# anhtu293/nndepth

Hardware: AMD Instinct MI355X
Metric: stereo pairs/sec at 544x960, 32 iters (RAFT-Stereo) (higher is better)
Workload: dtype f32 carried as 2 range-scaled fp16 pieces per operand (3 MFMA products, fp32 accumulate); 1 GPU; RAFT-Stereo base (ctx 64), 544x960, 32 iters, batch 1 per GPU, all 32 up_disp emitted; parallelism=single, launch=direct

## Files before the change

nndepth_amd/csrc/common.h:

```cpp
#pragma once
#include <hip/hip_runtime.h>
#include <atomic>
#include <cstdarg>
#include <cstdio>
#include "../../include/nndepth_amd.h"
#include "split_arith.h"

namespace nnd {

void set_error(const char* fmt, ...);

#define NND_HIP_CHECK(expr)                                                              \
    do {                                                                                 \
        hipError_t _e = (expr);                                                          \
        if (_e != hipSuccess) {                                                          \
            nnd::set_error("%s failed: %s (%s:%d)", #expr, hipGetErrorString(_e), __FILE__, __LINE__); \
            return NND_ERR_HIP;                                                          \
        }                                                                                \
    } while (0)

#define NND_LAUNCH_CHECK()                                                               \
    do {                                                                                 \
        hipError_t _e = hipGetLastError();                                               \
        if (_e != hipSuccess) {                                                          \
            nnd::set_error("kernel launch failed: %s (%s:%d)", hipGetErrorString(_e), __FILE__, __LINE__); \
            return NND_ERR_HIP;                                                          \
        }                                                                                \
    } while (0)

#define NND_REQUIRE(cond, ...)                                                           \
    do {                                                                                 \
        if (!(cond)) {                                                                   \
            nnd::set_error(__VA_ARGS__);                                                 \
            return NND_ERR_INVALID;                                                      \
        }                                                                                \
    } while (0)

#define NND_TRY(x)                           \
    do {                                     \
        if ((rc = (x)) != NND_OK) return rc; \
    } while (0)

template <class Desc>
static inline int check_desc(const Desc* d, unsigned allowed_flags, const char* name) {
    NND_REQUIRE(d, "%s: null descriptor", name);
    NND_REQUIRE(d->struct_size == (int32_t)sizeof(Desc), "%s: descriptor of %d bytes, this library expects %d (struct_size)", name,
                d->struct_size, (int)sizeof(Desc));
    NND_REQUIRE((d->flags & ~allowed_flags) == 0, "%s: unknown flags 0x%x", name, d->flags);
    return NND_OK;
}

struct Switches {
    bool no_fused_upsample, no_fused_lookup, no_fused_flow_branch, no_c4, agcl_v1, no_thin3d, corr_build_v1, corr_build_no_ksplit, igev_squeeze_v1, igev_squeeze_walk, no_folded_flow_head, no_conv1x1_stream,
        conv_verbose, debug_sync;
    int split_ny, split_ks, split_p;
    bool split_no_fast;
    bool no_merged_fb_lookup;
    int conv_p, conv_ks, conv_wco;
    int agcl_pb;
    bool lds_poison_on;
    unsigned lds_poison;
    int lds_slack;
    bool enc_no_c4;
    bool no_slab3d;
    int slab3d_rounds;
};
const Switches& switches();

static inline int raise_lds_limit(const void* kern, std::atomic<unsigned>& done, int bytes = 160 * 1024) {
    int dev = 0;
    NND_HIP_CHECK(hipGetDevice(&dev));
    const unsigned bit = 1u << (dev & 31);
    if (!(done.load(std::memory_order_relaxed) & bit)) {
        NND_HIP_CHECK(hipFuncSetAttribute(kern, hipFuncAttributeMaxDynamicSharedMemorySize, bytes));
        done.fetch_or(bit, std::memory_order_relaxed);
    }
    return NND_OK;
}

bool calibrating();
struct CalibScope {
    explicit CalibScope(bool on);
    ~CalibScope();
    CalibScope(const CalibScope&) = delete;
    CalibScope& operator=(const CalibScope&) = delete;
    bool on;
};
struct Act;
struct Lay;
int calib_amax_act(const Act& a, const Lay& lay, int B, int H, int W, const float* tail, hipStream_t s);
int calib_amax_flat(const float* x, int64_t n, const float* tail, hipStream_t s);
int calib_finish(float* blob, const int64_t* tail_offs, int n, int32_t* status_dev, hipStream_t s);

#ifdef __HIPCC__
__device__ __forceinline__ void fmac_scalar(float& acc, float a, float b) { asm("v_fmac_f32 %0, %1, %2" : "+v"(acc) : "v"(a), "v"(b)); }

__device__ __forceinline__ float relu_nan(float v) { return __builtin_elementwise_maximum(v, 0.f); }
__device__ __forceinline__ float clamp_nan(float v, float lo, float hi) {
    return __builtin_elementwise_minimum(__builtin_elementwise_maximum(v, lo), hi);
}
#endif

int to_tiled(const float* src, float* dst, int64_t dbs, int B, int C, int H, int W, hipStream_t s, int c0 = 0, bool c4 = false);
int from_tiled(const float* src, int64_t sbs, float* dst, int B, int C, int H, int W, hipStream_t s, int c0 = 0, bool c4 = false);

static inline int cdiv(int a, int b) { return (a + b - 1) / b; }
static inline int64_t cdiv64(int64_t a, int64_t b) { return (a + b - 1) / b; }

enum ConvEpilogue {
    EPI_LINEAR = 0,
    EPI_RELU = 1,
    EPI_GRU_ZR = 2,
    EPI_GRU_Q = 3,
    EPI_SCALE = 4,
    EPI_AFFINE = 5,
    EPI_SIGMOID_RANGE = 6,
    EPI_GELU = 7,
    EPI_HSWISH = 8
};

struct ConvLayer {
    int KH, KW, Cin, Cout, CI_T;
    int stride = 1;
    int arith = 0;
    bool range_scaled() const { return split_range_scaled(arith); }
    int64_t s_off = -1;
    int nchunks;
    int ncb;
    int64_t w_off, b_off;
    int64_t w_floats() const {
        return arith ? (int64_t)ncb * nchunks * KH * KW * arith * 256
                     : (int64_t)ncb * nchunks * KH * KW * CI_T * 32;
    }
    int64_t b_floats() const { return (int64_t)ncb * 32 + (range_scaled() ? 4 : 0); }
    double flops(int B, int H, int W) const { return 2.0 * B * H * W * (double)Cout * Cin * KH * KW; }
    int64_t tail_off() const { return b_off + (int64_t)ncb * 32; }
};

struct Act {
    float* ptr;
    int64_t bstride;
    int C;
};

struct ConvIO {
    Act src0, src1;
    Act out0, out1;
    Act aux0, aux1;
    Act bmap;
    int hidden = 0;
    float scale = 1.f;
    int Hin = 0, Win = 0;
    int flags = 0;
    bool src_tiled = false;
    bool dst_tiled = false;
    bool src_c4 = false;
    bool dst_c4 = false;
    int cout_need = 0;
    int force_ks = 0;
};

static inline bool conv_shape_built(int KH, int KW) { return (KH == 1 && (KW == 1 || KW == 5)) || (KW == 1 && KH == 5) || (KH == 3 && KW == 3); }

int conv_ci_t(int KH, int KW, int Cin, int stride = 1, int Cout = 0);

int launch_conv(const ConvLayer& L, const float* blob, const ConvIO& io, int epi,
                int B, int H, int W, hipStream_t stream);

void pack_conv(const ConvLayer& L, int nparts, const float* const* w, const float* const* b,
               const int* cout, float* blob, const int* ci_map = nullptr, int cin_src = 0);

bool conv_split_supported(int KH, int KW, int Cin, int stride, int arith, int Cout = 0);
int launch_conv_split(const ConvLayer& L, const float* blob, const ConvIO& io, int epi, int B, int H, int W, hipStream_t stream);
bool flow_branch_supported(const ConvLayer& f2, int fc);
int launch_flow_branch(const ConvLayer& f2, const float* blob, const float* w7t, const float* b7, const float* flow, int64_t fbs,
                       int fc, const ConvIO& io, int B, int H, int W, hipStream_t stream);
void pack_conv_split(const ConvLayer& L, int nparts, const float* const* w, const float* const* b, const int* cout, float* blob,
                     const int* ci_map, int cin_src);

bool thin3d_supported(int Cout, int stride);
bool slab3d_supported(int Cout, int C0, int C1, int stride, int arith);
int64_t slab3d_packed_floats(int Cout, int Ct, int stride);
void slab3d_pack(int Cout, int Ct, int stride, const float* w, const float* scale, const float* shift, float* out);
int slab3d_forward(int Cout, int C0, int C1, int stride, const float* packed, const float* x0, const float* x1, float* y, int N, int D,
                   int H, int W, float slope, hipStream_t s);
int64_t thin3d_packed_floats(int Cout, int Ct);
void thin3d_pack(int Cout, int Ct, const float* w, const float* scale, const float* shift, float* out);
int thin3d_forward(int Cout, int C0, int C1, int stride, const float* packed, const float* x0, const float* x1, float* y, int N, int D,
                   int H, int W, float slope, hipStream_t s);

int corr1d_lookup_launch(const float* pyr, const float* coords, float* out, int B, int H, int W, int num_levels,
                         int radius, hipStream_t stream, bool tiled);
int group_lookup_flat_launch(const float* pyr, const float* coords, float* out, int B, int G, int H, int W, int num_levels, int radius,
                             hipStream_t stream, bool tiled);
int igev_lookup_launch(const float* feat_pyramid, const float* geo_pyramid, const float* coords, float* out, int B, int G, int H,
                       int W, int num_levels, int radius, hipStream_t stream, bool tiled);
int convex_upsample_launch(const float* flow, const float* mask, float* out, int B, int C, int H, int W, int rate,
                           hipStream_t stream, bool tiled);

int agcl_iter_launch(const float* f1, const float* f2, const float* flow, float* warped, float* out, int N, int C, int H,
                     int W, int small_patch, hipStream_t s, bool tiled);
int agcl_offset_launch(const float* f1, const float* f2, const float* flow, const float* extra, float* out, int N, int C, int H,
                       int W, int small_patch, hipStream_t s, bool tiled);
int agcl_check(const char* what, int N, int C, int H, int W);
bool agcl_offset_cl_supported(int C);
int agcl_offset_cl_launch(const float* f1c, const float* f2c, const float* flow, const float* extra, float* out, int N, int C,
                          int H, int W, int small_patch, hipStream_t s, bool tiled);
int nchw_to_nhwc_launch(const float* in, float* out, int N, int C, int P, hipStream_t s);
int lookup_convc1_launch(const float* pyr, const float* geo, int G, const float* coords, const ConvLayer& L, const float* blob,
                         float* c1, int64_t c1_bs, int B, int H, int W, int num_levels, int radius, hipStream_t stream, bool c1_c4);
bool flow_branch_lookup_supported(int arith);
int flow_branch_lookup_launch(const ConvLayer& f2, const float* blob, const float* w7t, const float* b7, const float* flow, int64_t fbs,
                              int fc, const ConvIO& io, const float* pyr, const float* coords, const ConvLayer& Lc1, float* c1,
                              int64_t c1_bs, int B, int H, int W, int num_levels, int radius, hipStream_t stream, bool c1_c4);
bool igev_lookup_convc1_il_supported(int G, int num_levels, int radius);
int igev_lookup_convc1_il_launch(const float* il, int G, const float* coords, const ConvLayer& L, const float* blob, float* c1,
                                 int64_t c1_bs, int B, int H, int W, int num_levels, int radius, hipStream_t stream, bool c1_c4);
struct MaskUpFlowHead {
    const float* x;
    long xbs;
    int hid;
    const float* w;
    const float* bias;
    const float* coords_in;
    float *coords_out, *flow_out, *delta_out;
    float* hx_flow;
    long hx_bs;
    int hx_pm;
    int absolute;
};

bool mask_upsample_supported(int rate, int cin, int flow_channels);
bool mask_upsample_fold_supported(const ConvLayer& L, int hid);
int mask_upsample_launch(const ConvLayer& L, const float* blob, const float* x, int64_t xbs, const float* flow, float* out,
                         int B, int H, int W, int rate, hipStream_t stream, bool tiled, int flow_channels = 1, bool x_c4 = false,
                         const MaskUpFlowHead* fh = nullptr);

}
```

nndepth_amd/csrc/conv_epilogue.h:

```cpp
#pragma once
#include "common.h"
#include "layout.h"

namespace nnd {

typedef float f32x16 __attribute__((ext_vector_type(16)));

struct ConvArgs {
    const float* src0;
    const float* src1;
    long bs0, bs1;
    int c0, c1;
    const float* wpk;
    const float* bias;
    float* out0;
    float* out1;
    long obs0, obs1;
    const float* aux0;
    const float* aux1;
    long abs0, abs1;
    const float* bmap;
    long bmbs;
    Lay ls, ld;
    int H, W, Cout, nchunks, epi, hidden;
    int Hin, Win;
    int tiles_x, wco, ks, npos, ngroups;
    int flags;
    const float* cscale;
    float scale;
    int dbg_stamp;
};

__device__ __forceinline__ float exp_acc(float x) {
    const float L2E = 1.44269504088896341f;
    x = clamp_nan(x, -87.0f, 88.0f);
    const float t = x * L2E;
    const float r = fmaf(x, 1.92596299e-8f, fmaf(x, L2E, -t));
    const float e = __builtin_amdgcn_exp2f(t);
    return fmaf(e, r * 0.693147180559945f, e);
}
__device__ __forceinline__ float rcp_acc(float d) {
    float y = __builtin_amdgcn_rcpf(d);
    return fmaf(fmaf(-d, y, 1.0f), y, y);
}
__device__ __forceinline__ float sigmoidf_(float v) { return rcp_acc(1.0f + exp_acc(-v)); }
__device__ __forceinline__ float tanhf_(float v) {
    const float ax = fabsf(v);
    const float big = fmaf(-2.0f, rcp_acc(exp_acc(2.0f * ax) + 1.0f), 1.0f);
    const float x2 = ax * ax;
    const float small = ax * fmaf(x2, fmaf(x2, 0.133333333f, -0.333333333f), 1.0f);
    return copysignf(ax < 0.04f ? small : big, v);
}

template <int P>
__device__ __forceinline__ void conv_epilogue_planar(const ConvArgs& a, const f32x16 (&acc)[P], const int cb, const int b, const int h2,
                                                     const int reg0, const int nreg, const int (&ys)[P], const int (&xs)[P]) {
    const int H = a.H, W = a.W;
    const long DP = a.ld.plane;
    const int epi = a.epi;
    float bias_r[16];
#pragma unroll
    for (int reg = 0; reg < 16; ++reg) {
        const int co = cb * 32 + (reg & 3) + 8 * (reg >> 2) + 4 * h2;
        bias_r[reg] = (!a.bmap && reg >= reg0 && reg < reg0 + nreg && co < a.Cout) ? a.bias[co] : 0.f;
    }
#pragma unroll
    for (int pp = 0; pp < P; ++pp) {
        const int y = ys[pp], x = xs[pp];
        const bool pix_ok = (y < H && x < W);
        const long pix = pix_ok ? pix_off(a.ld, y, x) : 0;
        float h_r[16], z_r[16];
        if (a.bmap) {
#pragma unroll
            for (int reg = 0; reg < 16; ++reg) {
                const int co = cb * 32 + (reg & 3) + 8 * (reg >> 2) + 4 * h2;
                const bool ok = pix_ok && reg >= reg0 && reg < reg0 + nreg && co < a.Cout;
                bias_r[reg] = ok ? a.bmap[b * a.bmbs + co * DP + pix] : 0.f;
            }
        }
        if (epi == EPI_AFFINE) {
#pragma unroll
            for (int reg = 0; reg < 16; ++reg) {
                const int co = cb * 32 + (reg & 3) + 8 * (reg >> 2) + 4 * h2;
                const bool ok = pix_ok && reg >= reg0 && reg < reg0 + nreg && co < a.Cout;
                z_r[reg] = ok ? a.cscale[co] : 0.f;
                h_r[reg] = (ok && a.aux0) ? a.aux0[b * a.abs0 + co * DP + pix] : 0.f;
            }
        }
        if (epi == EPI_GRU_ZR || epi == EPI_GRU_Q) {
#pragma unroll
            for (int reg = 0; reg < 16; ++reg) {
                const int co = cb * 32 + (reg & 3) + 8 * (reg >> 2) + 4 * h2;
                const bool ok = pix_ok && reg >= reg0 && reg < reg0 + nreg && co < a.Cout;
                h_r[reg] = 0.f;
                z_r[reg] = 0.f;
                if (epi == EPI_GRU_Q) {
                    if (ok) {
                        h_r[reg] = a.aux0[b * a.abs0 + co * DP + pix];
                        z_r[reg] = a.aux1[b * a.abs1 + co * DP + pix];
                    }
                } else if (ok && co >= a.hidden) {
                    h_r[reg] = a.aux0[b * a.abs0 + (co - a.hidden) * DP + pix];
                }
            }
        }
        if (!pix_ok) continue;
#pragma unroll
        for (int reg = 0; reg < 16; ++reg) {
            if (reg < reg0 || reg >= reg0 + nreg) continue;
            const int co = cb * 32 + (reg & 3) + 8 * (reg >> 2) + 4 * h2;
            if (co >= a.Cout) continue;
            const float v = acc[pp][reg] + bias_r[reg];
            if (epi == EPI_RELU) {
// ... 111 lines not shown
                }
                r0[i] = o0;
                r1[i] = o1;
            }
            const bool to1 = epi == EPI_GRU_ZR && co0 >= a.hidden;
            float* d0 = to1 ? a.out1 + b * a.obs1 + (long)(co0 - a.hidden) * DP + pix : a.out0 + b * a.obs0 + (long)co0 * DP + pix;
            float rr[4];
#pragma unroll
            for (int i = 0; i < 4; ++i) rr[i] = to1 ? r1[i] : r0[i];
            if (full) {
                *reinterpret_cast<float4*>(d0) = make_float4(rr[0], rr[1], rr[2], rr[3]);
                if (epi == EPI_GRU_Q && a.out1) *reinterpret_cast<float4*>(a.out1 + b * a.obs1 + (long)co0 * DP + pix) = make_float4(r1[0], r1[1], r1[2], r1[3]);
            } else {
#pragma unroll
                for (int i = 0; i < 4; ++i)
                    if (co0 + i < a.Cout) {
                        d0[i] = rr[i];
                        if (epi == EPI_GRU_Q && a.out1) a.out1[b * a.obs1 + (long)co0 * DP + pix + i] = r1[i];
                    }
            }
        }
    }
}

template <int P, int NG>
struct EpiOpsC4 {
    float4 bm[P][NG], hv[P][NG], zv[P][NG];
    float4 scale4[NG];
    long pix[P];
    bool pix_ok[P];
};

template <int P, int NG>
__device__ __forceinline__ void epi_c4_load(const ConvArgs& a, const int cb, const int b, const int h2, const int q0,
                                            const int (&ys)[P], const int (&xs)[P], EpiOpsC4<P, NG>& e) {
    const long DP = a.ld.plane;
    const int epi = a.epi;
    auto ld4 = [](const float* p) { return *reinterpret_cast<const float4*>(p); };
    float4 bias4[NG];
#pragma unroll
    for (int j = 0; j < NG; ++j) {
        const int co0 = cb * 32 + 8 * (q0 + j) + 4 * h2;
        float bv[4], sv[4];
#pragma unroll
        for (int i = 0; i < 4; ++i) {
            bv[i] = (!a.bmap && co0 + i < a.Cout) ? a.bias[co0 + i] : 0.f;
            sv[i] = (epi == EPI_AFFINE && co0 + i < a.Cout) ? a.cscale[co0 + i] : 0.f;
        }
        bias4[j] = make_float4(bv[0], bv[1], bv[2], bv[3]);
        e.scale4[j] = make_float4(sv[0], sv[1], sv[2], sv[3]);
    }
#pragma unroll
    for (int pp = 0; pp < P; ++pp) {
        const int y = ys[pp], x = xs[pp];
        const bool pix_ok = (y < a.H && x < a.W);
        const long pix = pix_ok ? pix_off(a.ld, y, x) : 0;
        e.pix_ok[pp] = pix_ok;
        e.pix[pp] = pix;
#pragma unroll
        for (int j = 0; j < NG; ++j) {
            const int co0 = cb * 32 + 8 * (q0 + j) + 4 * h2;
            const bool ok = pix_ok && co0 + 3 < a.Cout;
            const float4 zero = make_float4(0.f, 0.f, 0.f, 0.f);
            e.bm[pp][j] = bias4[j];
            e.hv[pp][j] = zero;
            e.zv[pp][j] = zero;
            if (a.bmap && ok) e.bm[pp][j] = ld4(a.bmap + b * a.bmbs + (long)co0 * DP + pix);
            if (epi == EPI_AFFINE) {
                if (a.aux0 && ok) e.hv[pp][j] = ld4(a.aux0 + b * a.abs0 + (long)co0 * DP + pix);
            } else if (epi == EPI_GRU_Q) {
                if (ok) {
                    e.hv[pp][j] = ld4(a.aux0 + b * a.abs0 + (long)co0 * DP + pix);
                    e.zv[pp][j] = ld4(a.aux1 + b * a.abs1 + (long)co0 * DP + pix);
                }
            } else if (epi == EPI_GRU_ZR) {
                if (ok && co0 >= a.hidden) e.hv[pp][j] = ld4(a.aux0 + b * a.abs0 + (long)(co0 - a.hidden) * DP + pix);
            }
        }
    }
}

template <int P, int NG>
__device__ __forceinline__ void epi_c4_store(const ConvArgs& a, const float4 (&cacc)[P][NG], const int cb, const int b, const int h2,
                                             const int q0, const EpiOpsC4<P, NG>& e) {
    const long DP = a.ld.plane;
    const int epi = a.epi;
    auto get = [](const float4& v, int i) { return i == 0 ? v.x : (i == 1 ? v.y : (i == 2 ? v.z : v.w)); };
#pragma unroll
    for (int pp = 0; pp < P; ++pp) {
        if (!e.pix_ok[pp]) continue;
        const long pix = e.pix[pp];
#pragma unroll
        for (int j = 0; j < NG; ++j) {
            const int co0 = cb * 32 + 8 * (q0 + j) + 4 * h2;
            if (co0 >= a.Cout) continue;
            const bool full = co0 + 3 < a.Cout;
            float r0[4], r1[4];
#pragma unroll
            for (int i = 0; i < 4; ++i) {
                const float ac = get(cacc[pp][j], i);
                const float v = ac + get(e.bm[pp][j], i);
                float o0 = v, o1 = 0.f;
                if (epi == EPI_RELU) o0 = relu_nan(v);
                else if (epi == EPI_SCALE) o0 = a.scale * v;
                else if (epi == EPI_SIGMOID_RANGE) o0 = a.scale * (sigmoidf_(v) - 0.5f) * 2.0f;
                else if (epi == EPI_AFFINE) {
                    float y2 = fmaf(ac, get(e.scale4[j], i), get(e.bm[pp][j], i));
                    if (a.flags & 4) y2 = y2 > 0.f ? y2 : a.scale * y2;
                    if (a.flags & 1) y2 = relu_nan(y2);
                    if (a.aux0) y2 = get(e.hv[pp][j], i) + y2;
                    if (a.flags & 2) y2 = relu_nan(y2);
                    o0 = y2;
                } else if (epi == EPI_GRU_ZR) {
                    const float sg = sigmoidf_(v);
                    o0 = sg;
                    o1 = sg * get(e.hv[pp][j], i);
                } else if (epi == EPI_GRU_Q) {
                    const float qq = tanhf_(v);
                    o0 = fmaf(get(e.zv[pp][j], i), qq, (1.0f - get(e.zv[pp][j], i)) * get(e.hv[pp][j], i));
                    o1 = o0;
                }
                r0[i] = o0;
                r1[i] = o1;
            }
            const bool to1 = epi == EPI_GRU_ZR && co0 >= a.hidden;
            float* d0 = to1 ? a.out1 + b * a.obs1 + (long)(co0 - a.hidden) * DP + pix : a.out0 + b * a.obs0 + (long)co0 * DP + pix;
            float rr[4];
#pragma unroll
            for (int i = 0; i < 4; ++i) rr[i] = to1 ? r1[i] : r0[i];
            if (full) {
                *reinterpret_cast<float4*>(d0) = make_float4(rr[0], rr[1], rr[2], rr[3]);
                if (epi == EPI_GRU_Q && a.out1) *reinterpret_cast<float4*>(a.out1 + b * a.obs1 + (long)co0 * DP + pix) = make_float4(r1[0], r1[1], r1[2], r1[3]);
            } else {
#pragma unroll
                for (int i = 0; i < 4; ++i)
                    if (co0 + i < a.Cout) {
                        d0[i] = rr[i];
                        if (epi == EPI_GRU_Q && a.out1) a.out1[b * a.obs1 + (long)co0 * DP + pix + i] = r1[i];
                    }
            }
        }
    }
}

template <int P>
__device__ __forceinline__ void conv_epilogue(const ConvArgs& a, const f32x16 (&acc)[P], const int cb, const int b, const int h2,
                                              const int reg0, const int nreg, const int (&ys)[P], const int (&xs)[P]) {
    if (a.ld.ci == 4) conv_epilogue_c4<P>(a, acc, cb, b, h2, reg0, nreg, ys, xs);
    else conv_epilogue_planar<P>(a, acc, cb, b, h2, reg0, nreg, ys, xs);
}

}
```

nndepth_amd/csrc/conv_launch.h:

```cpp
#pragma once
#include "common.h"
#include "conv_epilogue.h"
#include "layout.h"

#include <cstring>

namespace nnd {

inline int conv_check_io(const char* who, const ConvLayer& L, const ConvIO& io, int epi, int H, int W, int* Hin, int* Win) {
    NND_REQUIRE(io.src0.C + io.src1.C == L.Cin, "%s: source channels %d+%d != Cin %d", who, io.src0.C, io.src1.C, L.Cin);
    NND_REQUIRE(L.stride == 1 || L.stride == 2, "%s: stride %d not supported", who, L.stride);
    *Hin = io.Hin > 0 ? io.Hin : H, *Win = io.Win > 0 ? io.Win : W;
    NND_REQUIRE(H == (*Hin + L.stride - 1) / L.stride && W == (*Win + L.stride - 1) / L.stride,
                "%s: output %dx%d does not match input %dx%d at stride %d", who, H, W, *Hin, *Win, L.stride);
    NND_REQUIRE(!io.src_c4 || (io.src_tiled && io.src0.C % 4 == 0 && io.src1.C % 4 == 0), "%s: c4 sources need channel counts %% 4 == 0", who);
    NND_REQUIRE(!io.dst_c4 || (io.dst_tiled && (L.Cout % 4 == 0 || (!io.bmap.ptr && !io.aux0.ptr && !io.aux1.ptr && !io.out1.ptr))),
                "%s: c4 destination with per-pixel operands needs Cout %% 4 == 0", who);
    NND_REQUIRE(epi != EPI_AFFINE || L.s_off >= 0, "%s: EPI_AFFINE needs a packed scale vector", who);
    return NND_OK;
}

inline void conv_fill_args(const ConvLayer& L, const float* blob, const ConvIO& io, int epi, int H, int W, int Hin, int Win, ConvArgs* out) {
    ConvArgs& a = *out;
    memset(&a, 0, sizeof(a));
    a.src0 = io.src0.ptr; a.bs0 = io.src0.bstride; a.c0 = io.src0.C;
    a.src1 = io.src1.ptr; a.bs1 = io.src1.bstride; a.c1 = io.src1.C;
    a.wpk = blob + L.w_off; a.bias = blob + L.b_off;
    a.out0 = io.out0.ptr; a.obs0 = io.out0.bstride;
    a.out1 = io.out1.ptr; a.obs1 = io.out1.bstride;
    a.aux0 = io.aux0.ptr; a.abs0 = io.aux0.bstride;
    a.aux1 = io.aux1.ptr; a.abs1 = io.aux1.bstride;
    a.bmap = io.bmap.ptr; a.bmbs = io.bmap.bstride;
    a.ls = make_lay(Hin, Win, io.src_tiled, io.src_c4);
    a.ld = make_lay(H, W, io.dst_tiled, io.dst_c4);
    a.H = H; a.W = W; a.Hin = Hin; a.Win = Win; a.Cout = L.Cout; a.nchunks = L.nchunks; a.epi = epi; a.hidden = io.hidden; a.flags = io.flags;
    a.cscale = L.s_off >= 0 ? blob + L.s_off : nullptr; a.scale = io.scale;
}

template <class CanStage>
inline bool conv_restrict_cout(const ConvLayer& L, int cout_need, int* ny, int* wco, CanStage can_stage) {
    const int nb = cdiv(cout_need, 32);
    if (cout_need <= 0 || nb >= L.ncb) return false;
    const int w = cdiv(nb, *ny), rows = cdiv(nb, *wco);
    if (w < *wco && can_stage(w)) {
        *wco = w;
        *ny = cdiv(nb, w);
        return true;
    }
    if (rows >= *ny) return false;
    *ny = rows;
    return true;
}

}
```

nndepth_amd/csrc/conv_mfma.hip:

```cpp
#include "conv_launch.h"

#include <cmath>
#include <cstdlib>
#include <cstring>
#include <type_traits>

namespace nnd {

#ifndef NND_INTERLEAVE
#define NND_INTERLEAVE 0
#endif

#ifndef NND_SC
#define NND_SC 8
#endif
__host__ __device__ constexpr int patch_stride(int PC, int SC) {
    int s = SC;
    while (s < PC) s += 2 * SC;
    return s;
}

#ifdef NND_DBG_STAMPS
__device__ unsigned long long g_stamps[4096 * 8];
#define NND_STAMP(i)                                                                                   \
// ... 411 lines not shown
                double unit = (double)cdiv(L.nchunks, ks) * P;
                double per_simd = std::ceil(waves / 1024.0);
                double t = (per_simd <= occ) ? per_simd * unit : std::ceil(waves / (1024.0 * occ)) * occ * unit;
                t *= std::ceil(wco * ks / 4.0) * 4.0 / (wco * ks);
                if (waves <= 1024.0) t *= 1.10;
                t *= 1.0 + 0.02 * (4 - wco);
                t *= 1.0 - 0.02 * (P - 1);
                t *= 1.0 + 0.01 * (ks - 1);
                if (t < best) {
                    best = t;
                    *out = {P, wco, ks, tx, ty, npos, ngroups, ne, lds};
                    found = true;
                }
            }
        }
    }
    return found;
}

template <int KH, int KW, int CI_T, int P, int NE, int STR = 1>
static int launch_one(const ConvArgs& a, const TileCfg& cfg, hipStream_t stream) {
    auto kern = conv_mfma_kernel<KH, KW, CI_T, P, NE, STR>;
    if (cfg.lds > 64 * 1024) {
        static std::atomic<unsigned> raised{0};
        if (int rc = raise_lds_limit(reinterpret_cast<const void*>(kern), raised)) return rc;
    }
    hipLaunchKernelGGL(kern, cfg.grid, cfg.block, cfg.lds, stream, a);
    return NND_OK;
}

template <int KH, int KW, int CI_T>
static int launch_shape(const ConvArgs& a, const TileCfg& cfg, hipStream_t stream) {
    return cfg.ne <= 8 ? launch_one<KH, KW, CI_T, 1, 8>(a, cfg, stream) : launch_one<KH, KW, CI_T, 1, 16>(a, cfg, stream);
}

static bool plan_tile(const ConvLayer& L, const ConvIO& io, int epi, int B, int H, int W, TileCfg* cfg) {
    if (!pick_tile(L, io.src0.C, io.src1.C, B, H, W, cfg, io.force_ks)) return false;
    cfg->stream1x1 = !switches().no_conv1x1_stream && L.KH == 1 && L.KW == 1 && L.stride == 1 && io.src1.C == 0 && io.src_tiled &&
                     (!io.dst_c4 || L.Cout % 4 == 0) && !io.bmap.ptr && (L.Cin == 64 || L.Cin == 96 || L.Cin == 128) &&
                     (epi == EPI_LINEAR || epi == EPI_RELU || epi == EPI_SCALE || epi == EPI_AFFINE);
    if (cfg->stream1x1) {
        cfg->grid = dim3((unsigned)cdiv64((long)L.ncb * cfg->tiles_x * cfg->tiles_y, 4), 1, B), cfg->block = dim3(256);
        return true;
    }
    auto groups = [&](int wco) { return 64 * wco * cfg->ks / cfg->npos; };
    int ny = cdiv(L.ncb, cfg->wco);
    cfg->restricted = conv_restrict_cout(L, io.cout_need, &ny, &cfg->wco,
                                         [&](int wco) { return groups(wco) > 0 && cdiv(cfg->ks * L.CI_T, groups(wco)) <= 16; });
    cfg->ngroups = groups(cfg->wco), cfg->ne = cdiv(cfg->ks * L.CI_T, cfg->ngroups);
    cfg->grid = dim3(cfg->tiles_x * cfg->tiles_y, ny, B), cfg->block = dim3(64 * cfg->wco * cfg->ks);
    return true;
}

static int check_tile_plan(const ConvLayer& L, const TileCfg& cfg) {
    const int SR_ = 32 / NND_SC, st = L.stride;
    const int PR_ = (SR_ - 1) * st + L.KH, PC_ = (cfg.P * NND_SC - 1) * st + L.KW;
    const size_t patch = (size_t)st * st * ((PR_ + st - 1) / st) * patch_stride((PC_ + st - 1) / st, NND_SC);
    NND_REQUIRE(cfg.lds >= ((size_t)2 * cfg.ks * L.CI_T * patch + 1) * sizeof(float) &&
                    (cfg.ks == 1 || cfg.lds >= (size_t)cfg.wco * cfg.ks * cfg.P * 1024 * sizeof(float)) && cfg.lds <= 160 * 1024,
                "conv: LDS plan %zu B does not cover the patch buffers / split-K tiles", cfg.lds);
    NND_REQUIRE(cfg.npos == PR_ * PC_ && cfg.npos * cfg.ngroups <= 64 * cfg.wco * cfg.ks && cfg.ngroups * cfg.ne >= cfg.ks * L.CI_T && cfg.ne <= 16,
                "conv: staging plan (%d positions x %d groups x %d) does not cover %d channels", cfg.npos, cfg.ngroups, cfg.ne, cfg.ks * L.CI_T);
    return NND_OK;
}

static void print_tile_plan(const ConvLayer& L, const ConvIO& io, const TileCfg& cfg) {
    if (cfg.stream1x1)
        fprintf(stderr, "[nnd] conv1x1_stream Cin=%d Cout=%d CI_T=%d: grid %ux1x%d%s\n", L.Cin, L.Cout, L.CI_T, cfg.grid.x, (int)cfg.grid.z,
                io.dst_c4 ? ", c4 destination" : "");
    else
        fprintf(stderr, "[nnd] conv %dx%d Cin=%d Cout=%d CI_T=%d: P=%d, wco=%d, ks=%d, ne=%d, grid %ux%ux%u, lds %zu B%s%s\n",
                L.KH, L.KW, L.Cin, L.Cout, L.CI_T, cfg.P, cfg.wco, cfg.ks, cfg.ne, cfg.grid.x, cfg.grid.y, cfg.grid.z, cfg.lds,
                io.cout_need > 0 ? (cfg.restricted ? ", restricted to the wanted output channels" : ", whole layer (not restrictable)") : "",
                L.stride == 2 ? ", stride 2" : "");
}

int launch_conv(const ConvLayer& L, const float* blob, const ConvIO& io, int epi, int B, int H, int W, hipStream_t stream) {
    if (L.arith != 0) {
        NND_REQUIRE(epi != EPI_GELU && epi != EPI_HSWISH, "conv: EPI_GELU / EPI_HSWISH are built on the exact fp32 kernel only");
        return launch_conv_split(L, blob, io, epi, B, H, W, stream);
    }
    int rc, Hin, Win;
    NND_TRY(conv_check_io("conv", L, io, epi, H, W, &Hin, &Win));
    NND_REQUIRE(io.src1.C == 0 || io.src0.C % L.CI_T == 0, "conv: first source (%d ch) must be a multiple of %d", io.src0.C, L.CI_T);
    NND_REQUIRE(!io.src_c4 || L.stride == 1, "conv: c4 sources need stride 1");
    NND_REQUIRE((long)(L.Cin + 2 * L.CI_T) * tiled_plane(Hin, Win) < (1L << 31), "conv: plane offsets exceed 32 bits");
    NND_REQUIRE((epi != EPI_GELU && epi != EPI_HSWISH) || (!io.dst_c4 && !io.out1.ptr && !io.bmap.ptr),
                "conv: EPI_GELU / EPI_HSWISH are built for a planar out0 only");
    TileCfg cfg;
    NND_REQUIRE(plan_tile(L, io, epi, B, H, W, &cfg),
                "conv: no tile configuration for %dx%d Cin=%d Cout=%d stride %d (NND_CONV_CFG p=%d ks=%d wco=%d, layer ks=%d)", L.KH, L.KW,
                L.Cin, L.Cout, L.stride, switches().conv_p, switches().conv_ks, switches().conv_wco, io.force_ks);
    NND_TRY(check_tile_plan(L, cfg));
    ConvArgs a;
    conv_fill_args(L, blob, io, epi, H, W, Hin, Win, &a);
    a.tiles_x = cfg.tiles_x; a.wco = cfg.wco; a.ks = cfg.ks; a.npos = cfg.npos; a.ngroups = cfg.ngroups;
    if (switches().conv_verbose) print_tile_plan(L, io, cfg);
    const int ntiles = cfg.tiles_x * cfg.tiles_y, KQ = L.nchunks * L.CI_T / 8, KH = L.KH, KW = L.KW, CI_T = L.CI_T;
    rc = NND_ERR_UNSUPPORTED;
    if (cfg.stream1x1) {
        rc = NND_OK;
        if (L.Cin == 64) launch_conv1x1_stream<8>(a, cfg.grid, ntiles, L.ncb, KQ, stream);
        else if (L.Cin == 96) launch_conv1x1_stream<12>(a, cfg.grid, ntiles, L.ncb, KQ, stream);
        else launch_conv1x1_stream<16>(a, cfg.grid, ntiles, L.ncb, KQ, stream);
    } else if (L.stride == 2) {
        if (KH == 3 && KW == 3 && CI_T == 16) rc = launch_one<3, 3, 16, 1, 16, 2>(a, cfg, stream);
        else if (KH == 1 && KW == 1 && CI_T == 16) rc = launch_one<1, 1, 16, 1, 16, 2>(a, cfg, stream);
        else set_error("conv %dx%d stride 2 CI_T=%d not instantiated", KH, KW, CI_T);
    } else if (KH == 1 && KW == 1 && CI_T == 128) rc = launch_shape<1, 1, 128>(a, cfg, stream);
    else if (KH == 1 && KW == 1 && CI_T == 32) rc = launch_shape<1, 1, 32>(a, cfg, stream);
    else if (KH == 3 && KW == 3 && CI_T == 32) rc = launch_shape<3, 3, 32>(a, cfg, stream);
    else if (KH == 3 && KW == 3 && CI_T == 16) rc = launch_shape<3, 3, 16>(a, cfg, stream);
    else if (KH == 1 && KW == 5 && CI_T == 32) rc = launch_shape<1, 5, 32>(a, cfg, stream);
    else if (KH == 5 && KW == 1 && CI_T == 32) rc = launch_shape<5, 1, 32>(a, cfg, stream);
    else if (KH == 1 && KW == 5 && CI_T == 64) rc = launch_shape<1, 5, 64>(a, cfg, stream);
    else if (KH == 5 && KW == 1 && CI_T == 64) rc = launch_shape<5, 1, 64>(a, cfg, stream);
    else set_error("conv %dx%d CI_T=%d not instantiated", KH, KW, CI_T);
    if (rc != NND_OK) return rc;
    NND_LAUNCH_CHECK();
    return NND_OK;
}

int conv_ci_t(int KH, int KW, int Cin, int stride, int Cout) {
    if (stride == 2) return 16;
    if (KH == 3 && KW == 3 && Cin <= 64) return 16;
    if (KH * KW == 5 && Cin >= 256 && Cout >= 256) return 64;
    return (KH == 1 && KW == 1 && Cin >= 128) ? 128 : 32;
}

void pack_conv(const ConvLayer& L, int nparts, const float* const* w, const float* const* bvec,
               const int* cout, float* blob, const int* ci_map, int cin_src) {
    if (L.arith != 0) return pack_conv_split(L, nparts, w, bvec, cout, blob, ci_map, cin_src);
    if (!ci_map) cin_src = L.Cin;
    const int NT = L.KH * L.KW, NQ = L.CI_T / 8;
    float* wp = blob + L.w_off;
    float* bp = blob + L.b_off;
    memset(wp, 0, sizeof(float) * L.w_floats());
    memset(bp, 0, sizeof(float) * L.b_floats());
    int co0 = 0;
    for (int part = 0; part < nparts; ++part) {
        for (int col = 0; col < cout[part]; ++col) {
            int co = co0 + col;
            int cb = co / 32, i = co % 32;
            bp[co] = bvec[part] ? bvec[part][col] : 0.f;
            for (int ci = 0; ci < L.Cin; ++ci) {
                int chunk = ci / L.CI_T, cl = ci % L.CI_T;
                int pair = cl / 2, h2 = cl % 2;
                int q = pair / 4, j = pair % 4;
                int lane = h2 * 32 + i;
                for (int t = 0; t < NT; ++t) {
                    size_t idx = (((((size_t)cb * L.nchunks + chunk) * NT + t) * NQ + q) * 64 + lane) * 4 + j;
                    wp[idx] = w[part][((size_t)col * cin_src + (ci_map ? ci_map[ci] : ci)) * NT + t];
                }
            }
        }
        co0 += cout[part];
    }
}

#ifdef NND_DBG_STAMPS
extern "C" int nnd_debug_read_stamps(unsigned long long* host, int n) {
    return hipMemcpyFromSymbol(host, HIP_SYMBOL(g_stamps), sizeof(unsigned long long) * n) == hipSuccess ? 0 : -1;
}
#endif
}
```

nndepth_amd/csrc/conv_split.hip:

```cpp
#include "conv_launch.h"
#include "conv_split_kernel.h"
#include "flow_branch.h"

#include <atomic>
#include <cmath>
#include <cstdlib>
#include <cstring>

namespace nnd {

namespace {
uint16_t f16_rn(float x) {
    const _Float16 h = (_Float16)x;
    uint16_t u;
    memcpy(&u, &h, 2);
    return u;
}
float f16_to_f(uint16_t u) {
    _Float16 h;
    memcpy(&h, &u, 2);
    return (float)h;
}
uint16_t bf16_rn(float x) {
    uint32_t u;
    memcpy(&u, &x, 4);
    if ((u & 0x7fffffffu) > 0x7f800000u) return (uint16_t)((u >> 16) | 0x40);
    u += 0x7fffu + ((u >> 16) & 1u);
    return (uint16_t)(u >> 16);
}
float bf16_to_f(uint16_t h) {
    const uint32_t u = (uint32_t)h << 16;
    float f;
    memcpy(&f, &u, 4);
    return f;
}

bool pick_split(const ConvLayer& L, int c0, int c1, int B, int H, int W, bool fast_ok, SplitCfg* out) {
    const int NS = L.arith, STR = L.stride;
    const int npos = split_patch(L.KH, L.KW, NS, STR).NPOS;
    const size_t subb = split_patch(L.KH, L.KW, NS, STR).SUBB;
    int tiles_x, ntiles = split_tiles(H, W, &tiles_x);
    int force_ny = switches().split_ny, force_ks = switches().split_ks, force_p = switches().split_p;
    const bool forced = force_ny > 0 || force_ks > 0 || force_p > 0;
    const long px_wgs2 = (long)cdiv(ntiles, 2) * B;
    bool rule = false;
    if (L.nchunks <= 4 && !forced && L.ncb <= SPLIT_MAX_WAVES) {
        force_ny = 1;
        while (force_ny < L.ncb && (L.ncb % force_ny != 0 || L.ncb / force_ny > 4)) ++force_ny;
        force_ks = 1;
        force_p = 2;
        rule = true;
    }
    bool try_ks2 = false;
    if (!rule && px_wgs2 >= 448 && !forced) {
        rule = true;
        force_ks = 1;
        force_ny = 1;
        force_p = 2;
        const int max_wco = L.nchunks >= 16 ? 4 : SPLIT_MAX_WAVES;
        while (force_ny < L.ncb && (L.ncb % force_ny != 0 || L.ncb / force_ny > max_wco)) ++force_ny;
        try_ks2 = px_wgs2 * force_ny * (L.ncb / force_ny) < 256 * SPLIT_MAX_WAVES / 2;
    }
    auto search = [&](int f_ny, int f_ks, int f_p) {
        double best = 1e30;
        bool found = false;
        for (int P : {2, 3, 4}) {
            if ((f_p > 0 && P != f_p) || (f_p <= 0 && P != 2)) continue;
            const long px_wgs = (long)cdiv(ntiles, P) * B;
            for (int ny = 1; ny <= L.ncb; ++ny) {
                if (L.ncb % ny != 0 || (f_ny > 0 && ny != f_ny)) continue;
                const int wco = L.ncb / ny;
                for (int ks : {1, 2, 4}) {
                    if (f_ks > 0 && ks != f_ks) continue;
                    const int waves = wco * ks;
                    if (waves > SPLIT_MAX_WAVES || ks > L.nchunks) continue;
                    if (c1 > 0 && c0 % (ks * 16) != 0) continue;
                    const bool fast = fast_ok && L.nchunks % ks == 0;
                    if (P > 2) continue;
                    if (STR == 2 && !fast) continue;
                    const int nu = split_staging_units(P, npos, ks, waves);
                    if (nu > 4 || (P == 3 && nu > 3)) continue;
                    size_t lds = (size_t)2 * ks * P * subb;
                    const size_t red = ks > 1 ? (size_t)waves * P * 4096 : 0;
                    if (red > lds) lds = red;
                    if (lds > 160 * 1024) continue;
                    const int max_waves = P > 2 ? 8 : SPLIT_MAX_WAVES;
                    int wg_per_cu = (int)((160 * 1024) / lds);
                    if (wg_per_cu > max_waves / waves) wg_per_cu = max_waves / waves;
                    if (wg_per_cu < 1) wg_per_cu = 1;
                    const double rounds = std::ceil((double)px_wgs * ny / (256.0 * wg_per_cu));
                    const double simd_waves = std::ceil(waves * wg_per_cu / 4.0);
                    double t = rounds * simd_waves * cdiv(L.nchunks, ks) * P / 2.0;
                    t *= 1.0 + 0.03 * (ks - 1);
                    t *= 1.0 + 0.02 * (4 - (wco < 4 ? wco : 4));
                    if (nu > 2 && P == 2) t *= 1.2;
                    if (t < best) {
                        best = t;
                        *out = {ny, wco, ks, P, ntiles, tiles_x, split_nu_variant(nu), fast, lds, STR};
                        found = true;
                    }
                }
            }
        }
        return found;
    };
    if (try_ks2 && search(force_ny, 2, force_p)) return true;
    if (search(force_ny, force_ks, force_p)) return true;
    return rule && search(-1, -1, -1);
}

bool restrict_split(const ConvLayer& L, int cout_need, SplitCfg* cfg) {
    const int npos = split_patch(L.KH, L.KW, L.arith, L.stride).NPOS;
    auto units = [&](int wco) { return split_staging_units(cfg->P, npos, cfg->ks, wco * cfg->ks); };
    if (!conv_restrict_cout(L, cout_need, &cfg->ny, &cfg->wco, [&](int wco) { return cfg->P == 2 && units(wco) <= 4; })) return false;
    cfg->nu = split_nu_variant(units(cfg->wco));
    return true;
}

bool split_fast_ok(const ConvLayer& L) { return !switches().split_no_fast || L.stride == 2; }
bool plan_split(const ConvLayer& L, const ConvIO& io, int B, int H, int W, SplitCfg* cfg) {
    if (!pick_split(L, io.src0.C, io.src1.C, B, H, W, split_fast_ok(L), cfg)) return false;
    cfg->restricted = restrict_split(L, io.cout_need, cfg);
    cfg->grid = dim3(cdiv(cfg->ntiles, cfg->P), cfg->ny, B), cfg->block = dim3(64 * cfg->wco * cfg->ks);
    return true;
}

void print_split_plan(const ConvLayer& L, const ConvIO& io, const SplitCfg& cfg) {
    fprintf(stderr, "[nnd] conv_split %dx%d Cin=%d Cout=%d pieces=%d: ny=%d, wco=%d, ks=%d, P=%d, nu=%d%s, grid %ux%ux%u, lds %zu B%s%s\n", L.KH,
            L.KW, L.Cin, L.Cout, L.arith, cfg.ny, cfg.wco, cfg.ks, cfg.P, cfg.nu, cfg.fast ? ", fast" : "", cfg.grid.x, cfg.grid.y, cfg.grid.z, cfg.lds,
            io.cout_need > 0 ? (cfg.restricted ? ", restricted to the wanted output channels" : ", whole layer (not restrictable)") : "",
            L.stride == 2 ? ", stride 2" : "");
}
}

extern template int launch_split_ns<1>(const ConvArgs&, const SplitCfg&, int, int, hipStream_t);
extern template int launch_split_ns<2>(const ConvArgs&, const SplitCfg&, int, int, hipStream_t);
extern template int launch_split_ns<3>(const ConvArgs&, const SplitCfg&, int, int, hipStream_t);

bool conv_split_supported(int KH, int KW, int Cin, int stride, int arith, int Cout) {
    if ((arith != 3 && arith != 2 && arith != 1) || (stride != 1 && stride != 2) || Cin % 16 != 0) return false;
    if (stride == 2) return ((KH == 3 && KW == 3) || (KH == 1 && KW == 1)) && Cout >= 96;
    return conv_shape_built(KH, KW);
}

int launch_conv_split(const ConvLayer& L, const float* blob, const ConvIO& io, int epi, int B, int H, int W, hipStream_t stream) {
    int rc, Hin, Win;
    NND_REQUIRE(conv_split_supported(L.KH, L.KW, L.Cin, L.stride, L.arith, L.Cout), "conv_split: %dx%d Cin=%d Cout=%d stride %d arith %d not built",
                L.KH, L.KW, L.Cin, L.Cout, L.stride, L.arith);
    NND_TRY(conv_check_io("conv_split", L, io, epi, H, W, &Hin, &Win));
    NND_REQUIRE(L.CI_T == 16 && L.nchunks * 16 == L.Cin, "conv_split: layer was not planned for 16-channel chunks");
    NND_REQUIRE(L.stride == 1 || io.src1.C == 0, "conv_split: stride 2 is built for one source");
    NND_REQUIRE((long)(L.Cin + 64) * tiled_plane(Hin, Win) < (1L << 31), "conv_split: plane offsets exceed 32 bits");
    SplitCfg cfg;
    NND_REQUIRE(plan_split(L, io, B, H, W, &cfg),
                "conv_split: no configuration for %dx%d Cin=%d (%d+%d) Cout=%d stride %d (NND_SPLIT_CFG ny=%d ks=%d P=%d%s)", L.KH, L.KW,
                L.Cin, io.src0.C, io.src1.C, L.Cout, L.stride, switches().split_ny, switches().split_ks, switches().split_p,
                split_fast_ok(L) ? "" : ", NND_SPLIT_NO_FAST");
    ConvArgs a;
    conv_fill_args(L, blob, io, epi, H, W, Hin, Win, &a);
    a.tiles_x = cfg.tiles_x; a.wco = cfg.wco; a.ks = cfg.ks; a.npos = cfg.ntiles;
#ifdef NND_DBG_STAMPS
    {
        static std::atomic<int> launches{0};
        static const int only = getenv("NND_DBG_STAMP_LAUNCH") ? atoi(getenv("NND_DBG_STAMP_LAUNCH")) : -1;
        const int idx = launches.fetch_add(1);
        a.dbg_stamp = only < 0 || idx == only;
    }
#endif
    if (calibrating() && split_range_scaled(L.arith))
        for (const Act* src : {&io.src0, &io.src1}) NND_TRY(calib_amax_act(*src, a.ls, B, Hin, Win, blob + L.tail_off(), stream));
    if (switches().conv_verbose) print_split_plan(L, io, cfg);
    rc = L.arith == 3   ? launch_split_ns<3>(a, cfg, L.KH, L.KW, stream)
         : L.arith == 2 ? launch_split_ns<2>(a, cfg, L.KH, L.KW, stream)
                        : launch_split_ns<1>(a, cfg, L.KH, L.KW, stream);
    NND_REQUIRE(rc != NND_ERR_UNSUPPORTED, "conv_split: shape %dx%d P=%d nu=%d %s is not instantiated", L.KH, L.KW, cfg.P, cfg.nu, cfg.fast ? "fast" : "generic");
    if (rc != NND_OK) return rc;
    NND_LAUNCH_CHECK();
    return NND_OK;
}

void pack_conv_split(const ConvLayer& L, int nparts, const float* const* w, const float* const* bvec, const int* cout, float* blob,
                     const int* ci_map, int cin_src) {
    if (!ci_map) cin_src = L.Cin;
    const int NT = L.KH * L.KW, NS = L.arith;
    uint16_t* wp = reinterpret_cast<uint16_t*>(blob + L.w_off);
    float* bp = blob + L.b_off;
    memset(wp, 0, sizeof(float) * L.w_floats());
    memset(bp, 0, sizeof(float) * L.b_floats());
    const bool f16 = split_range_scaled(NS);
    float wscale = 1.f;
    if (f16) {
        float wmax = 0.f;
        for (int part = 0; part < nparts; ++part)
            for (int col = 0; col < cout[part]; ++col)
                for (int ci = 0; ci < L.Cin; ++ci)
                    for (int t = 0; t < NT; ++t) {
                        const float v = std::fabs(w[part][((size_t)col * cin_src + (ci_map ? ci_map[ci] : ci)) * NT + t]);
                        if (std::isfinite(v) && v > wmax) wmax = v;
                    }
        int e = 0;
        if (wmax > 0.f) std::frexp(wmax, &e);
        const int s = wmax > 0.f ? 14 - e : 0;
        wscale = std::ldexp(1.f, s);
        float* tail = bp + L.ncb * 32;
        tail[SPLIT_TAIL_OSCALE] = std::ldexp(1.f, -(s + SPLIT_F16_XSHIFT));
        tail[SPLIT_TAIL_XSCALE] = std::ldexp(1.f, SPLIT_F16_XSHIFT);
        tail[SPLIT_TAIL_AMAX] = 0.f;
        tail[SPLIT_TAIL_WSINV] = std::ldexp(1.f, -s);
    }
    int co0 = 0;
    for (int part = 0; part < nparts; ++part) {
        for (int col = 0; col < cout[part]; ++col) {
            const int co = co0 + col, cb = co / 32, i = co % 32;
            bp[co] = bvec[part] ? bvec[part][col] : 0.f;
            for (int ci = 0; ci < L.Cin; ++ci) {
                const int chunk = ci / 16, cl = ci % 16, h = cl / 8, j = cl % 8, lane = h * 32 + i;
                for (int t = 0; t < NT; ++t) {
                    float res = w[part][((size_t)col * cin_src + (ci_map ? ci_map[ci] : ci)) * NT + t] * wscale;
                    for (int s = 0; s < NS; ++s) {
                        const uint16_t piece = f16 ? f16_rn(res) : bf16_rn(res);
                        res -= f16 ? f16_to_f(piece) : bf16_to_f(piece);
                        wp[((((((size_t)cb * L.nchunks + chunk) * NT + t) * NS + s) * 64 + lane) * 8) + j] = piece;
                    }
                }
            }
        }
        co0 += cout[part];
    }
}

template <int FC, int NS>
static int launch_fb(const FlowBranchArgs& a, dim3 grid, dim3 block, hipStream_t stream) {
    auto kern = flow_branch_kernel<FC, NS>;
    static std::atomic<unsigned> raised{0};
    if (int rc = raise_lds_limit(reinterpret_cast<const void*>(kern), raised)) return rc;
    const size_t lds = (size_t)(fb_lds_bytes<FC, NS>()) + switches().lds_slack;
    hipLaunchKernelGGL(kern, grid, block, lds, stream, a);
    return NND_OK;
}

bool flow_branch_supported(const ConvLayer& f2, int fc) {
    return (f2.arith == 3 || f2.arith == 2 || f2.arith == 1) && f2.KH == 3 && f2.KW == 3 && f2.Cin == FB_C1 && f2.Cout == 64 && f2.stride == 1 && (fc == 1 || fc == 2);
}
// ... 41 lines not shown
```

nndepth_amd/csrc/conv_split_kernel.h:

```cpp
#pragma once
#include "common.h"
#include "conv_epilogue.h"
#include "layout.h"
#include "split_arith.h"

#include <type_traits>
#include <utility>

namespace nnd {

#ifndef NND_SPLIT_BSLOTS
#define NND_SPLIT_BSLOTS 2
#endif

#ifdef NND_DBG_STAMPS
static __device__ unsigned long long g_split_stamps[4096 * 8];
#define NND_SSTAMP(i)                                                                                  \
    do {                                                                                               \
        if (threadIdx.x == 0 && a.dbg_stamp) {                                                         \
            const unsigned lin_ = blockIdx.x + gridDim.x * (blockIdx.y + gridDim.y * blockIdx.z);      \
            if (lin_ < 4096) g_split_stamps[lin_ * 8 + (i)] = __builtin_amdgcn_s_memrealtime();        \
        }                                                                                              \
    } while (0)
#define NND_SCLOCK(i)                                                                                  \
    do {                                                                                               \
        if (threadIdx.x == 0 && a.dbg_stamp) {                                                         \
            const unsigned lin_ = blockIdx.x + gridDim.x * (blockIdx.y + gridDim.y * blockIdx.z);      \
            if (lin_ < 4096) g_split_stamps[lin_ * 8 + (i)] = __builtin_amdgcn_s_memtime();            \
        }                                                                                              \
    } while (0)
#else
#define NND_SSTAMP(i)
#define NND_SCLOCK(i)
#endif
#if defined(NND_DBG_STAMPS) && defined(NND_DBG_PROLOGUE)
#undef NND_SCLOCK
#define NND_SCLOCK(i)
#define NND_PSTAMP(i) NND_SSTAMP(i)
#else
#define NND_PSTAMP(i)
#endif

__host__ __device__ constexpr int split_pos_bytes(int NS) { return NS * 32 + 16; }
__host__ __device__ constexpr int split_row_bytes(int PC, int NS) {
    int rb = (PC * split_pos_bytes(NS) + 15) / 16;
    while (rb % 16 != 8) ++rb;
    return rb * 16;
}

__device__ __forceinline__ int lane_pixel(int l31) {
    const bool g0 = (l31 < 4) || (l31 >= 12 && l31 < 16) || (l31 >= 20 && l31 < 28);
    const int idx = g0 ? (l31 < 4 ? l31 : (l31 < 16 ? l31 - 8 : l31 - 12)) : (l31 < 12 ? l31 - 4 : (l31 < 20 ? l31 - 8 : l31 - 16));
    return (g0 ? 0 : 16) + idx;
}

__host__ __device__ constexpr int split_gcd(int a, int b) { return b == 0 ? a : split_gcd(b, a % b); }

template <int N, typename F, int... I>
__device__ __forceinline__ void split_static_for_impl(F&& f, std::integer_sequence<int, I...>) {
    (f(std::integral_constant<int, I>{}), ...);
}
template <int N, typename F>
__device__ __forceinline__ void split_static_for(F&& f) {
    split_static_for_impl<N>(static_cast<F&&>(f), std::make_integer_sequence<int, N>{});
}

struct SplitPatch {
    int PRI, PCI, NPH, PRP, PCP, NPOS, PS, ROWB, PHB, SUBB;
};
__host__ __device__ constexpr SplitPatch split_patch(int KH, int KW, int NS, int STR) {
    const int PRI = 3 * STR + KH, PCI = 7 * STR + KW;
    const int NPH = STR == 1 ? 1 : (KH * KW == 1 ? 1 : 4);
    const int PRP = STR == 1 ? PRI : (KH == 1 ? 4 : (PRI + 1) / 2);
    const int PCP = STR == 1 ? PCI : (KW == 1 ? 8 : (PCI + 1) / 2);
    const int NPOS = STR == 1 ? PRI * PCI : (KH * KW == 1 ? 32 : PRI * PCI);
    const int ROWB = split_row_bytes(PCP, NS);
    return {PRI, PCI, NPH, PRP, PCP, NPOS, split_pos_bytes(NS), ROWB, PRP * ROWB, NPH * PRP * ROWB};
}
template <int KH, int KW, int NS, int STR>
struct SplitGeom {
    static constexpr SplitPatch G = split_patch(KH, KW, NS, STR);
    static constexpr int PRI = G.PRI, PCI = G.PCI, NPH = G.NPH, PRP = G.PRP, PCP = G.PCP, NPOS = G.NPOS;
    static constexpr int PS = G.PS, ROWB = G.ROWB, PHB = G.PHB, SUBB = G.SUBB;
};
__host__ __device__ constexpr int split_staging_units(int P, int npos, int ks, int waves) { return (P * npos * 2 * ks + 64 * waves - 1) / (64 * waves); }
__host__ __device__ constexpr int split_nu_variant(int nu) { return nu <= 2 ? 2 : 4; }

__host__ __device__ constexpr int split_pipe_spu(int nunit, int nsteps, int ul) {
    int v = 1;
    while (v < nsteps && nunit - 1 - (nsteps + v - 1) / v < ul + 3) ++v;
    return v;
}
template <int NT, int P, int NU>
struct SplitPipe {
    static constexpr int NUNIT = NT * P, NSTEPS = NU * 4 + 3, UL = 1;
    static constexpr int SPU = split_pipe_spu(NUNIT, NSTEPS, UL), U0 = NUNIT - 1 - (NSTEPS + SPU - 1) / SPU;
    static constexpr bool ON = NT >= 5 && P == 2;
};

template <int KH, int KW, int NS, int P, int NU, bool FAST, bool SRC4, int AD_, int MAXT, int STR = 1>
__global__ void __launch_bounds__(MAXT) conv_split_kernel(ConvArgs a) {
    static_assert(STR == 1 || (FAST && (KH * KW == 9 || KH * KW == 1)), "stride 2: 3x3 / 1x1, FAST regime");
    using Geo = SplitGeom<KH, KW, NS, STR>;
    constexpr int NT = KH * KW, PH = KH / 2, PW = KW / 2;
    constexpr int PC = Geo::PCI, NPOS = Geo::NPOS;
#ifndef NND_SPLIT_NO_PIPE
    constexpr bool PIPE = FAST && SRC4 && SplitPipe<NT, P, NU>::ON && NS != 1;
#else
    constexpr bool PIPE = false;
#endif
    constexpr int PS = Geo::PS, ROWB = Geo::ROWB, SUBB = Geo::SUBB, PHB = Geo::PHB;
    extern __shared__ __attribute__((aligned(16))) unsigned char lds_raw[];
    NND_SSTAMP(0);

    const int tid = threadIdx.x, lane = tid & 63, nthreads = blockDim.x;
    const int wave = __builtin_amdgcn_readfirstlane(tid >> 6);
    const int wco = a.wco, ks = a.ks;
    const int cbi = wave % wco, kj = wave / wco;
    const int h2 = lane >> 5, l31 = lane & 31;
    const int pxl = lane_pixel(l31), r = pxl >> 3, c = pxl & 7;
    const int cb = blockIdx.y * wco + cbi;
    const bool active = cb * 32 < a.Cout;
    const int b = blockIdx.z;
    const int Hin = a.Hin, Win = a.Win;
    const long SP = a.ls.plane;
    const int SCH = ks * 16;
    float oscale = 1.f, xscale = 1.f;
    if constexpr (split_range_scaled(NS)) {
        const float* tail = a.bias + (((a.Cout + 31) >> 5) << 5);
        oscale = tail[SPLIT_TAIL_OSCALE];
        xscale = tail[SPLIT_TAIL_XSCALE];
    }

    int ty0[P], tx0[P];
#pragma unroll
    for (int pp = 0; pp < P; ++pp) {
        const int t = blockIdx.x * P + pp;
        const bool valid = t < a.npos;
        ty0[pp] = valid ? (t / a.tiles_x) * 4 : (1 << 20);
        tx0[pp] = valid ? (t % a.tiles_x) * 8 : 0;
    }

    const int nunits = P * NPOS * 2 * ks;
    int goff[NU], loff[NU], cho[NU];
    bool inimg[NU], own[NU];
#pragma unroll
    for (int i = 0; i < NU; ++i) {
        const int u = PIPE ? min(tid + i * nthreads, nunits - 1) : tid + i * nthreads;
        own[i] = u < nunits;
        const int pos = u % NPOS, rest = u / NPOS;
        const int pp = rest % P, oct = rest / P;
        int pr, pc, lpos;
        if constexpr (STR == 1) {
            pr = pos / PC;
            pc = pos - pr * PC;
            lpos = pr * ROWB + pc * PS;
        } else if constexpr (KH * KW == 1) {
            pr = (pos >> 3) * 2;
            pc = (pos & 7) * 2;
            lpos = (pos >> 3) * ROWB + (pos & 7) * PS;
        } else {
            pr = pos / PC;
            pc = pos - pr * PC;
            lpos = ((pr & 1) * 2 + (pc & 1)) * PHB + (pr >> 1) * ROWB + (pc >> 1) * PS;
        }
        int gy = 0, gx = 0;
#pragma unroll
        for (int q = 0; q < P; ++q)
            if (q == pp) {
                gy = ty0[q] * STR + pr - PH;
                gx = tx0[q] * STR + pc - PW;
            }
        inimg[i] = own[i] && gy >= 0 && gy < Hin && gx >= 0 && gx < Win;
        goff[i] = inimg[i] ? (int)pix_off(a.ls, gy, gx) : 0;
        loff[i] = (oct >> 1) * (P * SUBB) + pp * SUBB + lpos + (oct & 1) * 16;
        cho[i] = oct * 8;
        if constexpr (FAST) goff[i] = inimg[i] ? cho[i] * (int)SP + goff[i] : 0;
        if constexpr (PIPE) goff[i] = cho[i] * (int)SP + (int)pix_off(a.ls, min(max(gy, 0), Hin - 1), min(max(gx, 0), Win - 1));
    }

    NND_PSTAMP(5);
    f32x16 acc[P];
#pragma unroll
    for (int pp = 0; pp < P; ++pp)
#pragma unroll
        for (int i = 0; i < 16; ++i) acc[pp][i] = 0.f;

    const int nchunks = a.nchunks;
    const int nsuper = (nchunks + ks - 1) / ks;
    const uint4* wbase = reinterpret_cast<const uint4*>(a.wpk) + (size_t)(active ? cb : 0) * nchunks * (NT * NS * 64) + lane;
    float stage[NU][8];

    auto chunk_src = [&](int K, const float*& src, int& climit) {
        const int cbase = K * SCH;
        if constexpr (FAST) {
            const bool first = cbase < a.c0;
            const float* s0 = a.src0 + b * a.bs0 + (long)cbase * SP;
            const float* s1 = a.src1 + b * a.bs1 + (long)(cbase - a.c0) * SP;
            src = first ? s0 : s1;
            climit = SCH;
        } else if (cbase < a.c0) {
            src = a.src0 + b * a.bs0 + (long)cbase * SP;
            climit = a.c0 - cbase;
        } else {
            const int cc = cbase - a.c0;
            src = a.src1 + b * a.bs1 + (long)cc * SP;
            climit = a.c1 - cc;
        }
    };
    const bool c4s = FAST ? SRC4 : a.ls.ci == 4;
    auto load_unit = [&](int K, int i) {
        const float* src;
        int climit;
        chunk_src(K, src, climit);
        if constexpr (FAST && SRC4) {
#pragma unroll
            for (int g = 0; g < 2; ++g) {
                const float4 t = *reinterpret_cast<const float4*>(src + (unsigned)(goff[i] + ((PIPE || inimg[i]) ? 4 * g * (int)SP : 0)));
                stage[i][4 * g] = t.x; stage[i][4 * g + 1] = t.y; stage[i][4 * g + 2] = t.z; stage[i][4 * g + 3] = t.w;
            }
        } else if constexpr (FAST) {
            const int step = inimg[i] ? (int)SP : 0;
#pragma unroll
            for (int j = 0; j < 8; ++j) stage[i][j] = src[(unsigned)(goff[i] + j * step)];
        } else if (c4s) {
#pragma unroll
            for (int g = 0; g < 2; ++g) {
                const int ci = cho[i] + 4 * g;
                const float4 t = *reinterpret_cast<const float4*>(src + ((inimg[i] && ci < climit) ? (unsigned)(ci * (int)SP + goff[i]) : 0u));
                stage[i][4 * g] = t.x; stage[i][4 * g + 1] = t.y; stage[i][4 * g + 2] = t.z; stage[i][4 * g + 3] = t.w;
            }
        } else {
#pragma unroll
            for (int j = 0; j < 8; ++j) {
                const int ci = cho[i] + j;
                stage[i][j] = src[(inimg[i] && ci < climit) ? (unsigned)(ci * (int)SP + goff[i]) : 0u];
            }
        }
    };
    auto store_unit = [&](int K, int i) {
        const float* src;
        int climit;
        chunk_src(K, src, climit);
        unsigned char* buf = lds_raw + (K & 1) * (ks * P * SUBB);
        float v[8];
#pragma unroll
        for (int j = 0; j < 8; ++j) v[j] = (inimg[i] && (FAST || cho[i] + j < climit)) ? stage[i][j] : 0.f;
        uint4 pieces[NS];
        split_pieces<NS>(v, pieces, xscale);
        if (own[i]) {
#pragma unroll
            for (int s = 0; s < NS; ++s) *reinterpret_cast<uint4*>(buf + loff[i] + s * 32) = pieces[s];
        }
    };
    auto load_x = [&](int K) {
#pragma unroll
        for (int i = 0; i < NU; ++i) load_unit(K, i);
    };
    auto store_x = [&](int K) {
#pragma unroll
        for (int i = 0; i < NU; ++i) store_unit(K, i);
    };
    auto a_ptr = [&](int K) {
        int ch = K * ks + kj;
        ch = ch < nchunks ? ch : 0;
        return wbase + (size_t)ch * (NT * NS * 64);
    };
    auto load_a = [&](uint4 (&dst)[NS], const uint4* wc, int t) {
#pragma unroll
        for (int s = 0; s < NS; ++s) dst[s] = wc[(t * NS + s) * 64];
    };

    const int lane_base = kj * (P * SUBB) + r * ROWB + c * PS + h2 * 16;

    constexpr int AD = (AD_ < NT ? AD_ : NT), NA = AD + 1;
    uint4 abuf[NA][NS];
#pragma unroll
    for (int g = 0; g < AD; ++g) load_a(abuf[g], a_ptr(0), g);
    load_x(0);
    NND_PSTAMP(6);
    store_x(0);
    NND_PSTAMP(7);
    __syncthreads();
    NND_SSTAMP(1);
    NND_SCLOCK(5);

    uint4 bq2[2][NS];
    uint32_t pw[NU][NS][4];
    auto read_b2 = [&](const unsigned char* xb, int u, uint4 (&dst)[NS]) {
        const int t = u / P, pp = u % P;
        const int dy = t / KW, dx = t % KW;
        const int toff = STR == 1 ? dy * ROWB + dx * PS : ((dy & 1) * 2 + (dx & 1)) * PHB + (dy >> 1) * ROWB + (dx >> 1) * PS;
#pragma unroll
        for (int s = 0; s < NS; ++s) dst[s] = *reinterpret_cast<const uint4*>(xb + pp * SUBB + toff + s * 32);
    };
    auto micro = [&](int q, unsigned char* wbuf) {
        using PP = SplitPipe<NT, P, NU>;
        if (q >= PP::NSTEPS) return;
        if (q < NU * 4) {
            const int i = q / 4, pr = q % 4;
            if constexpr (NS == 2) {
                const float sc = inimg[i] ? xscale : 0.f;
                uint32_t hi, lo;
                asm("v_fma_mixlo_f16 %0, %2, %3, 0\n\t"
                    "v_fma_mixhi_f16 %0, %2, %4, 0\n\t"
                    "v_fma_mixlo_f16 %1, %2, %3, -%0 op_sel_hi:[0,0,1]\n\t"
                    "v_fma_mixhi_f16 %1, %2, %4, -%0 op_sel:[0,0,1] op_sel_hi:[0,0,1]"
                    : "=&v"(hi), "=&v"(lo)
                    : "v"(sc), "v"(stage[i][2 * pr]), "v"(stage[i][2 * pr + 1]));
                pw[i][0][pr] = hi;
                pw[i][1][pr] = lo;
            } else {
                float r0 = inimg[i] ? stage[i][2 * pr] : 0.f, r1 = inimg[i] ? stage[i][2 * pr + 1] : 0.f;
#pragma unroll
                for (int sp = 0; sp < NS; ++sp) {
                    typedef __bf16 v2 __attribute__((ext_vector_type(2)));
                    v2 v;
                    v[0] = (__bf16)r0; v[1] = (__bf16)r1;
                    r0 -= (float)v[0]; r1 -= (float)v[1];
                    pw[i][sp][pr] = __builtin_bit_cast(uint32_t, v);
                }
            }
        }
        const int w = q - 4;
        if (w >= 0 && w / 4 < NU && w % 4 < NS) {
#ifdef NND_SPLIT_NO_LDSW
            if (pw[w / 4][0][0] == 0x12345678u)
#endif
            *reinterpret_cast<uint4*>(wbuf + loff[w / 4] + (w % 4) * 32) =
                make_uint4(pw[w / 4][w % 4][0], pw[w / 4][w % 4][1], pw[w / 4][w % 4][2], pw[w / 4][w % 4][3]);
        }
    };
    auto chunk_pipe = [&](int K, auto par_c, auto more_c) {
        using PP = SplitPipe<NT, P, NU>;
        constexpr int par = decltype(par_c)::value;
        constexpr bool more = decltype(more_c)::value;
        constexpr int NUNIT = PP::NUNIT;
        const int BUFB = ks * P * SUBB;
        const uint4* wc = a_ptr(K);
        const uint4* wn = a_ptr(more ? K + 1 : K);
        const unsigned char* xb = lds_raw + (K & 1) * BUFB + lane_base;
        const unsigned char* xbn = lds_raw + ((K + 1) & 1) * BUFB + lane_base;
        unsigned char* wbuf = lds_raw + ((K + 1) & 1) * BUFB;
#pragma unroll
        for (int t = 0; t < NT; ++t) {
            uint4(&ac)[NS] = abuf[(par + t) % NA];
            uint4(&an)[NS] = abuf[(par + t + AD) % NA];
#ifndef NND_SPLIT_NO_ALOAD
            if (t + AD < NT) load_a(an, wc, t + AD);
            else load_a(an, wn, t + AD - NT);
#else
            for (int s = 0; s < NS; ++s) an[s] = ac[s];
#endif
#pragma unroll
            for (int pp = 0; pp < P; ++pp) {
                const int u = t * P + pp;
#ifndef NND_SPLIT_NO_BREAD
                if (u + 1 < NUNIT) read_b2(xb, u + 1, bq2[(u + 1) & 1]);
                else if (more) read_b2(xbn, 0, bq2[0]);
#endif
                __builtin_amdgcn_sched_barrier(0);
#ifndef NND_SPLIT_NO_MFMA
                split_mfma_step<NS>(ac, bq2[u & 1], acc[pp]);
#else
// ... 38 lines not shown
            for (int s = 0; s < NS; ++s)
                dst[s] = *reinterpret_cast<const uint4*>(xb + pp * SUBB + toff + s * 32);
        };
#pragma unroll
        for (int u = 0; u < NSLOT - 1 && u < NUNIT; ++u) read_b(u, bq[u]);
#pragma unroll
        for (int t = 0; t < NT; ++t) {
            uint4(&ac)[NS] = abuf[(par + t) % NA];
            uint4(&an)[NS] = abuf[(par + t + AD) % NA];
#ifndef NND_SPLIT_NO_ALOAD
            if (t + AD < NT) load_a(an, wc, t + AD);
            else load_a(an, wn, t + AD - NT);
#else
            for (int s = 0; s < NS; ++s) an[s] = ac[s];
#endif
#pragma unroll
            for (int pp = 0; pp < P; ++pp) {
                const int u = t * P + pp;
                if (u + NSLOT - 1 < NUNIT) read_b(u + NSLOT - 1, bq[(u + NSLOT - 1) % NSLOT]);
#ifndef NND_SPLIT_NO_PIN
                if constexpr (FAST) __builtin_amdgcn_sched_barrier(0);
#endif
#ifndef NND_SPLIT_NO_MFMA
                if constexpr (mine)
#else
                if (mine && acc[0][0] == 123.f)
#endif
                    split_mfma_step<NS>(ac, bq[u % NSLOT], acc[pp]);
#ifndef NND_SPLIT_NO_PIN
                if constexpr (FAST) __builtin_amdgcn_sched_barrier(0);
#endif
            }
        }
#ifndef NND_SPLIT_NO_STAGE
        if (more) store_x(K + 1);
#endif
        __syncthreads();
    };
    auto chunk = [&](int K, auto par_c) {
        if constexpr (FAST) {
            chunk_body(K, par_c, std::true_type{});
        } else {
            if (K * ks + kj < nchunks) chunk_body(K, par_c, std::true_type{});
            else chunk_body(K, par_c, std::false_type{});
        }
    };
    constexpr int STEP = NT % NA, PERIOD = NA / split_gcd(STEP, NA);
    if constexpr (PIPE) read_b2(lds_raw + lane_base, 0, bq2[0]);
    if constexpr (PIPE) {
        const int last = nsuper - 1;
        for (int K0 = 0; K0 < last; K0 += PERIOD)
            split_static_for<PERIOD>([&](auto j) {
                constexpr int jj = decltype(j)::value;
                if (jj == 0 || K0 + jj < last) chunk_pipe(K0 + jj, std::integral_constant<int, (jj * STEP) % NA>{}, std::true_type{});
            });
        split_static_for<PERIOD>([&](auto j) {
            constexpr int jj = decltype(j)::value;
            if (PERIOD == 1 || last % PERIOD == jj) chunk_pipe(last, std::integral_constant<int, (jj * STEP) % NA>{}, std::false_type{});
        });
    } else {
        for (int K0 = 0; K0 < nsuper; K0 += PERIOD)
            split_static_for<PERIOD>([&](auto j) {
                constexpr int jj = decltype(j)::value;
                if (jj == 0 || K0 + jj < nsuper) chunk(K0 + jj, std::integral_constant<int, (jj * STEP) % NA>{});
            });
    }

    NND_SSTAMP(2);
    NND_SCLOCK(6);
    if constexpr (split_range_scaled(NS)) {
#pragma unroll
        for (int pp = 0; pp < P; ++pp)
#pragma unroll
            for (int i = 0; i < 16; ++i) acc[pp][i] *= oscale;
    }
    int ys[P], xs[P];
#pragma unroll
    for (int pp = 0; pp < P; ++pp) {
        ys[pp] = ty0[pp] + r;
        xs[pp] = tx0[pp] + c;
    }
    float* red_all = reinterpret_cast<float*>(lds_raw);
    constexpr int TS = P * 1024;
    auto exchange = [&]() {
        if (active) {
            float* red = red_all + (size_t)(cbi * ks + kj) * TS + lane;
#pragma unroll
            for (int pp = 0; pp < P; ++pp)
#pragma unroll
                for (int reg = 0; reg < 16; ++reg) red[pp * 1024 + reg * 64] = acc[pp][reg];
        }
        __syncthreads();
    };
    auto finish_c4 = [&](auto ng_c) {
        constexpr int NG = decltype(ng_c)::value;
        const int q0 = kj * NG;
        EpiOpsC4<P, NG> eo;
#ifndef NND_SPLIT_NO_EPI
        if (active) epi_c4_load<P, NG>(a, cb, b, h2, q0, ys, xs, eo);
#endif
        exchange();
        if (!active) return;
        float4 cacc[P][NG];
#pragma unroll
        for (int pp = 0; pp < P; ++pp)
#pragma unroll
            for (int j = 0; j < NG; ++j) {
                float v[4];
#pragma unroll
                for (int i = 0; i < 4; ++i) {
                    const float* red = red_all + (size_t)(cbi * ks) * TS + pp * 1024 + (4 * (q0 + j) + i) * 64 + lane;
                    float sum = red[0];
#pragma unroll
                    for (int sl = 1; sl < 4 / NG; ++sl) sum += red[(size_t)sl * TS];
                    v[i] = sum;
                }
                cacc[pp][j] = make_float4(v[0], v[1], v[2], v[3]);
            }
        NND_SSTAMP(3);
#ifdef NND_SPLIT_NO_EPI
        if (cacc[0][0].x != 123.456f) return;
#endif
        epi_c4_store<P, NG>(a, cacc, cb, b, h2, q0, eo);
    };
    if (a.ld.ci == 4) {
        if (ks == 4) finish_c4(std::integral_constant<int, 1>{});
        else if (ks == 2) finish_c4(std::integral_constant<int, 2>{});
        else {
            if (!active) return;
            NND_SSTAMP(3);
#ifdef NND_SPLIT_NO_EPI
            if (acc[0][0] != 123.456f) return;
#endif
            conv_epilogue_c4<P>(a, acc, cb, b, h2, 0, 16, ys, xs);
        }
    } else {
        if (ks > 1) exchange();
        if (!active) return;
        const int nreg = 16 / ks, reg0 = kj * nreg;
        if (ks > 1) {
            const float* red = red_all + (size_t)(cbi * ks) * TS + lane;
#pragma unroll
            for (int pp = 0; pp < P; ++pp)
#pragma unroll
                for (int reg = 0; reg < 16; ++reg) {
                    if (reg < reg0 || reg >= reg0 + nreg) continue;
                    float sum = red[pp * 1024 + reg * 64];
                    for (int j = 1; j < ks; ++j) sum += red[(size_t)j * TS + pp * 1024 + reg * 64];
                    acc[pp][reg] = sum;
                }
        }
        NND_SSTAMP(3);
#ifdef NND_SPLIT_NO_EPI
        if (acc[0][0] != 123.456f) return;
#endif
        conv_epilogue_planar<P>(a, acc, cb, b, h2, reg0, nreg, ys, xs);
    }
#ifdef NND_DBG_STAMPS
    __builtin_amdgcn_s_waitcnt(0);
#endif
    NND_SSTAMP(4);
}

struct SplitCfg {
    int ny, wco, ks, P, ntiles, tiles_x, nu;
    bool fast;
    size_t lds;
    int stride;
    bool restricted;
    dim3 grid, block;
};

constexpr int SPLIT_MAX_WAVES = 12;

inline int split_tiles(int H, int W, int* tiles_x) { return (*tiles_x = cdiv(W, 8)) * cdiv(H, 4); }

template <int KH, int KW, int NS, int P, int NU, bool FAST, bool SRC4, int AD, int MAXT, int STR = 1>
int launch_split_kernel(const ConvArgs& a, dim3 grid, dim3 block, size_t lds, hipStream_t stream) {
    auto kern = conv_split_kernel<KH, KW, NS, P, NU, FAST, SRC4, AD, MAXT, STR>;
    if ((int)block.x > MAXT) {
        set_error("conv_split: %u threads exceed the %d-thread bound of this instantiation", block.x, MAXT);
        return NND_ERR_INVALID;
    }
    lds += switches().lds_slack;
    if (lds > 64 * 1024) {
        static std::atomic<unsigned> raised{0};
        if (int rc = raise_lds_limit(reinterpret_cast<const void*>(kern), raised)) return rc;
    }
    hipLaunchKernelGGL(kern, grid, block, lds, stream, a);
    return NND_OK;
}

template <int KH, int KW, int NS>
constexpr int split_fast_ad() {
#ifdef NND_SPLIT_FAST_AD
    return NND_SPLIT_FAST_AD;
#else
    return KH * KW == 9 ? 2 : (KH * KW == 5 ? (NS <= 2 ? 4 : 2) : 1);
#endif
}

template <int KH, int KW, int NS, bool FAST, bool SRC4, int STR>
int launch_split_nu(const ConvArgs& a, const SplitCfg& cfg, hipStream_t stream) {
    constexpr int AD = FAST ? split_fast_ad<KH, KW, NS>() : 1;
    if (split_nu_variant(cfg.nu) == 2) return launch_split_kernel<KH, KW, NS, 2, 2, FAST, SRC4, AD, 768, STR>(a, cfg.grid, cfg.block, cfg.lds, stream);
    return launch_split_kernel<KH, KW, NS, 2, 4, FAST, SRC4, AD, 768, STR>(a, cfg.grid, cfg.block, cfg.lds, stream);
}
template <int KH, int KW, int NS>
int launch_split_shape(const ConvArgs& a, const SplitCfg& cfg, hipStream_t stream) {
    if (cfg.P != 2) return NND_ERR_UNSUPPORTED;
    const bool src4 = a.ls.ci == 4;
    if (cfg.stride == 2) {
        if constexpr (KH * KW == 9 || KH * KW == 1) {
            if (!cfg.fast) return NND_ERR_UNSUPPORTED;
            return src4 ? launch_split_nu<KH, KW, NS, true, true, 2>(a, cfg, stream) : launch_split_nu<KH, KW, NS, true, false, 2>(a, cfg, stream);
        } else {
            return NND_ERR_UNSUPPORTED;
        }
    }
    if (!cfg.fast) return launch_split_nu<KH, KW, NS, false, false, 1>(a, cfg, stream);
    return src4 ? launch_split_nu<KH, KW, NS, true, true, 1>(a, cfg, stream) : launch_split_nu<KH, KW, NS, true, false, 1>(a, cfg, stream);
}

template <int NS>
int launch_split_ns(const ConvArgs& a, const SplitCfg& cfg, int KH, int KW, hipStream_t stream) {
    if (KH == 3 && KW == 3) return launch_split_shape<3, 3, NS>(a, cfg, stream);
    if (KH == 1 && KW == 5) return launch_split_shape<1, 5, NS>(a, cfg, stream);
    if (KH == 5 && KW == 1) return launch_split_shape<5, 1, NS>(a, cfg, stream);
    if (KH == 1 && KW == 1) return launch_split_shape<1, 1, NS>(a, cfg, stream);
    return NND_ERR_UNSUPPORTED;
}

}
```

nndepth_amd/csrc/error.cpp:

```cpp
#include "common.h"

#include <cstdlib>

namespace nnd {
static thread_local char g_err[512] = "";
void set_error(const char* fmt, ...) {
    va_list ap;
    va_start(ap, fmt);
    vsnprintf(g_err, sizeof(g_err), fmt, ap);
    va_end(ap);
}

static Switches g_sw;
static void load_switches() {
    Switches s{};
    auto on = [](const char* n) { return getenv(n) != nullptr; };
    s.no_fused_upsample = on("NND_NO_FUSED_UPSAMPLE");
    s.no_fused_lookup = on("NND_NO_FUSED_LOOKUP");
    s.no_fused_flow_branch = on("NND_NO_FUSED_FLOW_BRANCH");
    s.no_c4 = on("NND_NO_C4");
    s.agcl_v1 = on("NND_AGCL_V1");
    s.no_thin3d = on("NND_NO_THIN3D");
    s.corr_build_v1 = on("NND_CORR_BUILD_V1");
    s.corr_build_no_ksplit = on("NND_CORR_BUILD_NO_KSPLIT");
    s.igev_squeeze_v1 = on("NND_IGEV_SQUEEZE_V1");
    s.igev_squeeze_walk = on("NND_IGEV_SQUEEZE_WALK");
    s.no_folded_flow_head = on("NND_NO_FOLDED_FLOW_HEAD");
    s.no_conv1x1_stream = on("NND_NO_CONV1X1_STREAM");
    s.conv_verbose = on("NND_CONV_VERBOSE");
    s.debug_sync = on("NND_DEBUG_SYNC");
    s.split_ny = s.split_ks = s.split_p = -1;
    if (const char* e = getenv("NND_SPLIT_CFG")) sscanf(e, "%d,%d,%d", &s.split_ny, &s.split_ks, &s.split_p);
    s.split_no_fast = on("NND_SPLIT_NO_FAST");
    s.no_merged_fb_lookup = on("NND_NO_MERGED_FB_LOOKUP");
    s.conv_p = s.conv_ks = s.conv_wco = -1;
    if (const char* e = getenv("NND_CONV_CFG")) sscanf(e, "%d,%d,%d", &s.conv_p, &s.conv_ks, &s.conv_wco);
    if (const char* e = getenv("NND_CONV_P")) s.conv_p = atoi(e);
    s.agcl_pb = getenv("NND_AGCL_PB") ? atoi(getenv("NND_AGCL_PB")) : 0;
    s.lds_poison_on = on("NND_DEBUG_LDS_POISON");
    s.lds_poison = s.lds_poison_on ? (unsigned)strtoul(getenv("NND_DEBUG_LDS_POISON"), nullptr, 0) : 0u;
    s.lds_slack = getenv("NND_DEBUG_LDS_SLACK") ? atoi(getenv("NND_DEBUG_LDS_SLACK")) : 0;
    s.enc_no_c4 = on("NND_ENC_NO_C4");
    s.no_slab3d = on("NND_NO_SLAB3D");
    s.slab3d_rounds = getenv("NND_SLAB3D_ROUNDS") ? atoi(getenv("NND_SLAB3D_ROUNDS")) : 0;
    g_sw = s;
}
namespace {
struct SwitchInit {
    SwitchInit() { load_switches(); }
} g_switch_init;
}
const Switches& switches() { return g_sw; }
}

extern "C" {
int nnd_reload_switches(void) {
    nnd::load_switches();
    return NND_OK;
}
int nnd_version(void) { return NND_VERSION; }
const char* nnd_last_error(void) { return nnd::g_err; }
int nnd_device_count(void) {
    int n = 0;
    if (hipGetDeviceCount(&n) != hipSuccess) {
        (void)hipGetLastError();
        return 0;
    }
    return n;
}
}
```

nndepth_amd/csrc/mask_upsample.hip:

```cpp
#include "common.h"

#include <type_traits>
#include "layout.h"
#include "split_arith.h"

namespace nnd {

typedef float f32x16 __attribute__((ext_vector_type(16)));

#ifdef NND_DBG_STAMPS
__device__ unsigned long long g_mu_stamps[4096 * 8];
#define NND_MSTAMP(i)                                                                             \
    do {                                                                                          \
        if (threadIdx.x == 0 && blockIdx.x < 4096) g_mu_stamps[blockIdx.x * 8 + (i)] = __builtin_amdgcn_s_memrealtime(); \
    } while (0)
#else
#define NND_MSTAMP(i)
#endif

struct MaskUpArgs {
    const float* x;
    long xbs;
    const float* wpk;
    const float* bias;
    const float* flow;
    float* out;
    int H, W, tiles_x, fc;
    Lay lay;
    int x_c4;
    int lds_floats;
    MaskUpFlowHead fh;
};

template <int RATE, int CIN>
struct MaskUpCfg {
    static constexpr int COUT = 9 * RATE * RATE;
    static constexpr int NCB = (COUT + 31) / 32;
    static constexpr int CBW = NCB >= 12 ? 3 : 1;
    static constexpr int G = (NCB + CBW - 1) / CBW;
    static constexpr int NWAVES = 2 * G;
    static constexpr int NT = 64 * NWAVES;
    static constexpr int NST = CIN / 32;
    static constexpr int MT_STRIDE = 33;
    static constexpr int XS_FLOATS = CIN * 32 * 3 / 2;
    static constexpr int LDS_FLOATS = (XS_FLOATS > COUT * MT_STRIDE ? XS_FLOATS : COUT * MT_STRIDE) + 128;
};

template <int RATE, int CIN, int NS = 0, int FHW = 0>
__global__ void __launch_bounds__((MaskUpCfg<RATE, CIN>::NT + 64 * FHW)) mask_upsample_kernel(MaskUpArgs a) {
    constexpr bool SPLIT = NS != 0;
    using Cfg = MaskUpCfg<RATE, CIN>;
    constexpr int COUT = Cfg::COUT, NCB = Cfg::NCB, CBW = Cfg::CBW, G = Cfg::G, NT = Cfg::NT, NST = Cfg::NST;
    constexpr int CI_T = 128;
    constexpr int NCHUNK = CIN / CI_T;
    constexpr int MTS = Cfg::MT_STRIDE;
    static_assert(CIN % 128 == 0 && NST % 2 == 0, "CIN must be a multiple of 128");
    extern __shared__ float lds[];
    NND_MSTAMP(0);
    float* xs = lds;
    float* mt = lds;
    float* fp = lds + a.lds_floats - 128;

    const int tid = threadIdx.x, lane = tid & 63;
    const int wave = __builtin_amdgcn_readfirstlane(tid >> 6);
    const int g = wave % G, kj = wave / G;
    const int h2 = lane >> 5, l31 = lane & 31;
    const int tx0 = (blockIdx.x % a.tiles_x) * 8, ty0 = (blockIdx.x / a.tiles_x) * 4;
    const int b = blockIdx.z;
    const int H = a.H, W = a.W;
    const long HW = (long)H * W;
    const long XP = a.lay.plane;
    float oscale = 1.f, xscale = 1.f;
    if constexpr (split_range_scaled(NS)) {
        oscale = a.bias[Cfg::NCB * 32 + SPLIT_TAIL_OSCALE];
        xscale = a.bias[Cfg::NCB * 32 + SPLIT_TAIL_XSCALE];
    }

    float fh_state = 0.f, fh_bias = 0.f;
    auto fh_finish = [&](float* fbase, int t0) {
        if (t0 >= 60) return;
        const float* part = fbase + a.fh.hid * 105;
        const int pr = t0 / 10, pc = t0 % 10;
        const int y = ty0 + pr - 1, x = tx0 + pc - 1;
        float sum = 0.f;
#pragma unroll
        for (int sl = 0; sl < 16; ++sl) sum += part[sl * 64 + t0];
        sum += fh_bias;
        const bool in = y >= 0 && y < H && x >= 0 && x < W;
        const float cnew = fh_state + sum;
        const float fl = a.fh.absolute ? cnew : cnew - (float)x;
        fp[t0] = in ? fl : 0.f;
        if (in && pr >= 1 && pr <= 4 && pc >= 1 && pc <= 8) {
            const long pix = pix_off(a.lay, y, x);
            a.fh.delta_out[b * XP + pix] = sum;
            a.fh.coords_out[b * XP + pix] = cnew;
            a.fh.flow_out[b * XP + pix] = fl;
            a.fh.hx_flow[b * a.fh.hx_bs + pix * a.fh.hx_pm] = fl;
        }
    };
    constexpr int NQ4 = (CIN / 4 * 32 + NT - 1) / NT;
    float4 v4[SPLIT ? NQ4 : 1];
    if constexpr (SPLIT) {
        const float* src = a.x + b * a.xbs;
#pragma unroll
        for (int i = 0; i < NQ4; ++i) {
            const int e = min(tid, NT - 1) + i * NT;
            const int qd = e >> 5, px = e & 31;
            const int y = ty0 + (px >> 3), x = tx0 + (px & 7);
            const bool ok = e < CIN / 4 * 32 && y < H && x < W;
            if (a.x_c4) {
                v4[i] = *reinterpret_cast<const float4*>(src + (ok ? (unsigned)(qd * 4 * (int)XP + 4 * (int)pix_off(a.lay, y, x)) : 0u));
            } else {
                const unsigned o = ok ? (unsigned)(qd * 4 * (int)XP + (int)pix_off(a.lay, y, x)) : 0u;
                v4[i] = make_float4(src[o], src[ok ? o + (unsigned)XP : 0u], src[ok ? o + 2u * (unsigned)XP : 0u], src[ok ? o + 3u * (unsigned)XP : 0u]);
            }
        }
    }
    if constexpr (FHW > 0) {
        if (tid >= NT) {
            float* fbase = lds + Cfg::LDS_FLOATS;
            const int hid = a.fh.hid, fw_ = __builtin_amdgcn_readfirstlane((tid - NT) >> 6), cn = hid / FHW, c0 = fw_ * cn;
            float* patch = fbase;
            float* fw = fbase + hid * 96;
            const float* src = a.fh.x + b * a.fh.xbs;
            constexpr int NPL = 12, NWL = 5;
            const int total = 96 * (cn / 4), nwt = cn * 9;
            float4 pv[NPL];
            bool pok[NPL];
            float wreg[NWL];
#pragma unroll
            for (int k = 0; k < NWL; ++k) wreg[k] = a.fh.w[c0 * 9 + min(lane + 64 * k, nwt - 1)];
            if (tid - NT < 60) {
                fh_bias = a.fh.bias[0];
                const int y = ty0 + (tid - NT) / 10 - 1, x = tx0 + (tid - NT) % 10 - 1;
                if (y >= 0 && y < H && x >= 0 && x < W) fh_state = a.fh.coords_in[b * XP + pix_off(a.lay, y, x)];
            }
#pragma unroll
            for (int j = 0; j < NPL; ++j) {
                const int e = min(lane + 64 * j, total - 1);
                const int pos = e % 96, q = c0 / 4 + e / 96;
                const int gy = ty0 + pos / 12 - 2, gx = tx0 + pos % 12 - 2;
                pok[j] = gy >= 0 && gy < H && gx >= 0 && gx < W;
                const long off = pok[j] ? pix_off(a.lay, gy, gx) : 0;
                if (a.x_c4) pv[j] = *reinterpret_cast<const float4*>(src + (long)q * 4 * XP + 4 * off);
                else pv[j] = make_float4(src[(long)(4 * q) * XP + off], src[(long)(4 * q + 1) * XP + off], src[(long)(4 * q + 2) * XP + off], src[(long)(4 * q + 3) * XP + off]);
            }
            __builtin_amdgcn_s_barrier();
#pragma unroll
            for (int j = 0; j < NPL; ++j) {
                const int e = lane + 64 * j;
                if (e < total) {
                    float* pp = patch + (c0 + 4 * (e / 96)) * 96 + e % 96;
                    pp[0] = pok[j] ? pv[j].x : 0.f;
                    pp[96] = pok[j] ? pv[j].y : 0.f;
                    pp[192] = pok[j] ? pv[j].z : 0.f;
                    pp[288] = pok[j] ? pv[j].w : 0.f;
                }
            }
#pragma unroll
            for (int k = 0; k < NWL; ++k)
                if (lane + 64 * k < nwt) fw[c0 * 9 + lane + 64 * k] = wreg[k];
            __builtin_amdgcn_fence(__ATOMIC_RELEASE, "workgroup");
            __builtin_amdgcn_wave_barrier();
            __builtin_amdgcn_fence(__ATOMIC_ACQUIRE, "workgroup");
            {
                const int cps = hid / 16, s0 = c0 / cps;
                const int pos = min(lane, 59), po = (pos / 10) * 12 + pos % 10;
                float acc[4] = {0.f, 0.f, 0.f, 0.f};
                for (int cc = 0; cc < cps; ++cc) {
                    float xv[4][9];
#pragma unroll
                    for (int k = 0; k < 4; ++k) {
                        const float* pp = patch + ((s0 + k) * cps + cc) * 96 + po;
#pragma unroll
                        for (int t = 0; t < 9; ++t) xv[k][t] = pp[(t / 3) * 12 + t % 3];
                    }
                    float wv[4][9];
#pragma unroll
                    for (int k = 0; k < 4; ++k) {
                        const float* wk = fw + ((s0 + k) * cps + cc) * 9;
#pragma unroll
                        for (int t = 0; t < 9; ++t) wv[k][t] = wk[t];
                    }
#pragma unroll
                    for (int k = 0; k < 4; ++k)
#pragma unroll
                        for (int t = 0; t < 9; ++t) fmac_scalar(acc[k], wv[k][t], xv[k][t]);
                }
                float* part = fbase + hid * 105;
                if (lane < 60)
#pragma unroll
                    for (int k = 0; k < 4; ++k) part[(s0 + k) * 64 + pos] = acc[k];
            }
            __syncthreads();
            fh_finish(fbase, tid - NT);
            __syncthreads();
            __syncthreads();
            return;
        }
    }
    {
// ... 136 lines not shown
            const float* xb = xs + ((s0 + sl) * 32 + h2) * 32 + l31;
    #pragma unroll
            for (int pair = 0; pair < 16; ++pair) dst[pair] = xb[pair * 64];
        };
        load_a(ab[0], 0);
        load_b(bq[0], 0);
    #pragma unroll
        for (int u = 0; u < SPW * CBW; ++u) {
            const int sl = u / CBW, cbi = u % CBW;
            if (u + 1 < SPW * CBW) load_a(ab[(u + 1) & 1], u + 1);
            if (cbi == 0 && sl + 1 < SPW) load_b(bq[(sl + 1) & 1], sl + 1);
            __builtin_amdgcn_sched_barrier(0);
    #pragma unroll
            for (int pair = 0; pair < 16; ++pair) {
                const float4 av = ab[u & 1][pair / 4];
                const float as = (pair % 4 == 0) ? av.x : (pair % 4 == 1) ? av.y : (pair % 4 == 2) ? av.z : av.w;
                acc[cbi] = __builtin_amdgcn_mfma_f32_32x32x2f32(as, bq[sl & 1][pair], acc[cbi], 0, 0, 0);
            }
            __builtin_amdgcn_sched_barrier(0);
        }
}
    NND_MSTAMP(2);
    __syncthreads();

#pragma unroll
    for (int pass = 0; pass < 2; ++pass) {
        if (kj == pass) {
#pragma unroll
            for (int cbi = 0; cbi < CBW; ++cbi) {
                const int cb = g * CBW + cbi;
#pragma unroll
                for (int reg = 0; reg < 16; ++reg) {
                    const int co = cb * 32 + (reg & 3) + 8 * (reg >> 2) + 4 * h2;
                    if (cb < NCB && co < COUT) {
                        float* p = mt + co * MTS + l31;
                        *p = pass == 0 ? acc[cbi][reg] : *p + acc[cbi][reg];
                    }
                }
            }
        }
        __syncthreads();
    }

    NND_MSTAMP(3);
    constexpr int ROWLEN = 8 * RATE;
    constexpr int NITEM = 4 * RATE * ROWLEN;
    const long OW = (long)W * RATE;
    for (int e = tid; e < NITEM; e += NT) {
        const int seg = e / ROWLEN, within = e % ROWLEN;
        const int rr = seg / RATE, i = seg % RATE;
        const int c = within / RATE, j = within % RATE;
        const int px = rr * 8 + c;
        const int y = ty0 + rr, x = tx0 + c;
        float m[9];
        float mx = -INFINITY;
#pragma unroll
        for (int k = 0; k < 9; ++k) {
            const int co = k * RATE * RATE + i * RATE + j;
            m[k] = 0.25f * (mt[co * MTS + px] + a.bias[co]);
            mx = fmaxf(mx, m[k]);
        }
        float sum = 0.f;
#pragma unroll
        for (int k = 0; k < 9; ++k) {
            m[k] = expf(m[k] - mx);
            sum += m[k];
        }
#pragma unroll
        for (int k = 0; k < 9; ++k) m[k] = m[k] / sum;
        for (int f = 0; f < a.fc; ++f) {
            float o = 0.f;
#pragma unroll
            for (int k = 0; k < 9; ++k) o += m[k] * ((float)RATE * fp[f * 60 + (rr + k / 3) * 10 + c + k % 3]);
            if (y < H && x < W) a.out[((long)b * a.fc + f) * HW * RATE * RATE + ((long)y * RATE + i) * OW + (long)x * RATE + j] = o;
        }
    }
#ifdef NND_DBG_STAMPS
    __builtin_amdgcn_s_waitcnt(0);
#endif
    NND_MSTAMP(4);
}

constexpr int MU_FHW = 4;
template <int RATE, int CIN, int NS, int FHW>
static int launch_mu_fhw(MaskUpArgs a, int B, hipStream_t stream) {
    using Cfg = MaskUpCfg<RATE, CIN>;
    auto kern = mask_upsample_kernel<RATE, CIN, NS, FHW>;
    a.lds_floats = Cfg::LDS_FLOATS;
    const int fh_floats = a.fh.x ? a.fh.hid * (96 + 9) + 16 * 64 : 0;
    if (FHW > 0) a.lds_floats = Cfg::LDS_FLOATS + fh_floats + 128;
    const size_t lds = a.lds_floats * sizeof(float);
    if (lds > 64 * 1024) {
        static std::atomic<unsigned> raised{0};
        if (int rc = raise_lds_limit(reinterpret_cast<const void*>(kern), raised)) return rc;
    }
    dim3 grid(a.tiles_x * cdiv(a.H, 4), 1, B), block(Cfg::NT + 64 * FHW);
    hipLaunchKernelGGL(kern, grid, block, lds, stream, a);
    NND_LAUNCH_CHECK();
    return NND_OK;
}
template <int RATE, int CIN, int NS = 0>
static int launch_mu(const MaskUpArgs& a, int B, hipStream_t stream) {
    if (a.fh.x) {
        if constexpr (split_range_scaled(NS)) return launch_mu_fhw<RATE, CIN, NS, MU_FHW>(a, B, stream);
        else NND_REQUIRE(false, "mask_upsample: the folded flow head is built for the fp16x2 and fp16 arithmetics");
    }
    return launch_mu_fhw<RATE, CIN, NS, 0>(a, B, stream);
}

bool mask_upsample_fold_supported(const ConvLayer& L, int hid) { return split_range_scaled(L.arith) && hid % 16 == 0 && hid <= 128; }

bool mask_upsample_supported(int rate, int cin, int flow_channels) {
    return (flow_channels == 1 || flow_channels == 2) && ((rate == 8 && (cin == 256 || cin == 128)) || (rate == 4 && (cin == 256 || cin == 128)));
}

int mask_upsample_launch(const ConvLayer& L, const float* blob, const float* x, int64_t xbs, const float* flow, float* out,
                         int B, int H, int W, int rate, hipStream_t stream, bool tiled, int flow_channels, bool x_c4,
                         const MaskUpFlowHead* fh) {
    NND_REQUIRE(L.KH == 1 && L.KW == 1 && L.CI_T == (L.arith ? 16 : 128) && L.Cout == 9 * rate * rate && L.arith >= 0 && L.arith <= 3,
                "mask_upsample: layer shape / packing");
    NND_REQUIRE(mask_upsample_supported(rate, L.Cin, flow_channels), "mask_upsample: rate %d / Cin %d / %d flow channels not built",
                rate, L.Cin, flow_channels);
    MaskUpArgs a;
    a.x = x; a.xbs = xbs; a.wpk = blob + L.w_off; a.bias = blob + L.b_off; a.flow = flow; a.out = out;
    a.H = H; a.W = W; a.tiles_x = cdiv(W, 8); a.fc = flow_channels;
    a.lay = make_lay(H, W, tiled);
    a.x_c4 = (tiled && x_c4) ? 1 : 0;
    a.lds_floats = 0;
    a.fh = MaskUpFlowHead{};
    if (fh && fh->x) {
        NND_REQUIRE(flow_channels == 1 && mask_upsample_fold_supported(L, fh->hid) && fh->w && fh->bias && fh->coords_in && fh->coords_out && fh->flow_out &&
                        fh->delta_out && fh->hx_flow && fh->coords_in != fh->coords_out,
                    "mask_upsample: folded flow head needs one flow channel, hid %% 16 == 0 and distinct old / new state buffers");
        a.fh = *fh;
    }
    if (L.arith == 3) {
        if (rate == 8 && L.Cin == 256) return launch_mu<8, 256, 3>(a, B, stream);
        if (rate == 8 && L.Cin == 128) return launch_mu<8, 128, 3>(a, B, stream);
        if (rate == 4 && L.Cin == 256) return launch_mu<4, 256, 3>(a, B, stream);
        return launch_mu<4, 128, 3>(a, B, stream);
    }
    if (split_range_scaled(L.arith)) {
        if (calibrating()) {
            const Act xa{const_cast<float*>(x), xbs, L.Cin};
            if (int rc = calib_amax_act(xa, make_lay(H, W, tiled, x_c4), B, H, W, blob + L.tail_off(), stream)) return rc;
        }
        if (L.arith == 1) {
            if (rate == 8 && L.Cin == 256) return launch_mu<8, 256, 1>(a, B, stream);
            if (rate == 8 && L.Cin == 128) return launch_mu<8, 128, 1>(a, B, stream);
            if (rate == 4 && L.Cin == 256) return launch_mu<4, 256, 1>(a, B, stream);
            return launch_mu<4, 128, 1>(a, B, stream);
        }
        if (rate == 8 && L.Cin == 256) return launch_mu<8, 256, 2>(a, B, stream);
        if (rate == 8 && L.Cin == 128) return launch_mu<8, 128, 2>(a, B, stream);
        if (rate == 4 && L.Cin == 256) return launch_mu<4, 256, 2>(a, B, stream);
        return launch_mu<4, 128, 2>(a, B, stream);
    }
    if (rate == 8 && L.Cin == 256) return launch_mu<8, 256>(a, B, stream);
    if (rate == 8 && L.Cin == 128) return launch_mu<8, 128>(a, B, stream);
    if (rate == 4 && L.Cin == 256) return launch_mu<4, 256>(a, B, stream);
    return launch_mu<4, 128>(a, B, stream);
}

#ifdef NND_DBG_STAMPS
extern "C" int nnd_debug_read_mu_stamps(unsigned long long* host, int n) {
    return hipMemcpyFromSymbol(host, HIP_SYMBOL(g_mu_stamps), sizeof(unsigned long long) * n) == hipSuccess ? 0 : -1;
}
#endif

}
```

nndepth_amd/csrc/update_block.hip:

```cpp
#include "common.h"
#include "conv_layer.h"
#include "layout.h"

#include <cstdlib>
#include <cstring>
#include <vector>

namespace nnd {

enum ConvId { C_C1 = 0, C_C2, C_F2, C_CV, C_ZR1X, C_Q1X, C_ZR2X, C_Q2X, C_FHM, C_M2, C_LOOP_COUNT,
              C_ZR1 = C_LOOP_COUNT, C_Q1, C_ZR2, C_Q2, C_ZR1C, C_Q1C, C_ZR2C, C_Q2C, C_COUNT };
static const char* kConvNames[C_COUNT] = {"encoder.convc1", "encoder.convc2", "encoder.convf2", "encoder.conv",
                                          "gru.convz1+convr1[h,motion]", "gru.convq1[rh,motion]", "gru.convz2+convr2[h,motion]",
                                          "gru.convq2[rh,motion]", "flow_head.conv1+mask.0", "mask.2",
                                          "gru.convz1+convr1", "gru.convq1", "gru.convz2+convr2", "gru.convq2",
                                          "gru.convz1+convr1[inp]", "gru.convq1[inp]", "gru.convz2+convr2[inp]", "gru.convq2[inp]"};

struct Plan {
    nnd_update_block_desc d;
    bool sep;
    int num_tensors;
    ConvLayer L[C_COUNT];
    int64_t f1_w, f1_b;
    int64_t f1_wt;
    int64_t fc2_w, fc2_b;
    int64_t total;
};

static ConvLayer mk(int KH, int KW, int Cin, int Cout, int64_t* off, int arith = 0) {
    return make_conv_layer(KH, KW, Cin, Cout, 1, arith, 0, false, off);
}

static size_t fc2_lds_bytes(int hid, int fc) { return (size_t)(hid * 64 + fc * hid * 9 + 16 * fc * 32) * sizeof(float); }

static int make_plan(const nnd_update_block_desc* d, Plan* p) {
    if (int rc = check_desc(d, NND_FLAG_CALIBRATE | NND_FLAG_LAST_UPSAMPLE_ONLY, "update_block")) return rc;
    const int hid = d->hidden_dim, ctx = d->context_dim, cp = d->cor_planes, fc = d->flow_channels, mc = d->mask_channels;
    NND_REQUIRE(hid > 0 && hid % 32 == 0, "update_block: hidden_dim %d must be a positive multiple of 32", hid);
    NND_REQUIRE(ctx > 0 && ctx % 8 == 0, "update_block: context_dim %d must be a positive multiple of 8", ctx);
    NND_REQUIRE(cp > 0 && (fc == 1 || fc == 2) && mc > 0 && mc % 9 == 0, "update_block: bad cor_planes/flow_channels/mask_channels");
    NND_REQUIRE(fc2_lds_bytes(hid, fc) <= 64 * 1024,
                "update_block: hidden_dim %d with %d flow channel(s) is not supported: flow_head.conv2 would stage %zu bytes of LDS (at most 65536)",
                hid, fc, fc2_lds_bytes(hid, fc));
    NND_REQUIRE(d->gru_kind == 0 || d->gru_kind == 1, "update_block: gru_kind must be 0 (sep_conv) or 1 (conv_gru)");
    NND_REQUIRE(d->arithmetic >= 0 && d->arithmetic <= 3,
                "update_block: arithmetic must be 0 (fp32 MFMA), 3 (bf16x3 split), 2 (fp16x2 split) or 1 (fp16, one piece)");
    const unsigned split_mask = d->split_layers ? (unsigned)d->split_layers : ~0u;
    auto ar = [&](int id) { return (d->arithmetic != 0 && ((split_mask >> id) & 1u)) ? d->arithmetic : 0; };
    p->d = *d;
    p->sep = d->gru_kind == 0;
    p->num_tensors = p->sep ? 30 : 24;
    int64_t off = 0;
    const int gin = hid + ctx + hid;
    p->L[C_C1] = mk(1, 1, cp, 256, &off, ar(C_C1));
    p->L[C_C2] = mk(3, 3, 256, 192, &off, ar(C_C2));
    p->f1_w = off; off += (int64_t)128 * fc * 49;
    p->f1_b = off; off += 128;
    p->f1_wt = off; off += (int64_t)128 * fc * 49;
    p->L[C_F2] = mk(3, 3, 128, 64, &off, ar(C_F2));
    p->L[C_CV] = mk(3, 3, 256, hid - fc, &off, ar(C_CV));
    for (int pass = 0; pass < (p->sep ? 2 : 1); ++pass) {
        const int kh = p->sep ? (pass == 0 ? 1 : 5) : 3, kw = p->sep ? (pass == 0 ? 5 : 1) : 3;
        const int zr = pass == 0 ? C_ZR1 : C_ZR2, q = pass == 0 ? C_Q1 : C_Q2;
        p->L[zr] = mk(kh, kw, gin, 2 * hid, &off, ar(zr));
        p->L[q] = mk(kh, kw, gin, hid, &off, ar(q));
        p->L[zr - C_ZR1 + C_ZR1X] = mk(kh, kw, 2 * hid, 2 * hid, &off, ar(zr - C_ZR1 + C_ZR1X));
        p->L[q - C_ZR1 + C_ZR1X] = mk(kh, kw, 2 * hid, hid, &off, ar(q - C_ZR1 + C_ZR1X));
        p->L[zr - C_ZR1 + C_ZR1C] = mk(kh, kw, ctx, 2 * hid, &off, ar(zr - C_ZR1 + C_ZR1C));
        p->L[q - C_ZR1 + C_ZR1C] = mk(kh, kw, ctx, hid, &off, ar(q - C_ZR1 + C_ZR1C));
    }
    if (!p->sep)
        for (int base : {(int)C_ZR1X, (int)C_ZR1, (int)C_ZR1C}) {
            p->L[base + 2] = p->L[base];
            p->L[base + 3] = p->L[base + 1];
        }
    p->L[C_FHM] = mk(3, 3, hid, 3 * hid, &off, ar(C_FHM));
    p->fc2_w = off; off += (int64_t)fc * hid * 9;
    p->fc2_b = off; off += 4;
    p->L[C_M2] = mk(1, 1, 2 * hid, mc, &off, ar(C_M2));
    p->total = off;
    return NND_OK;
}

static int refuse_last_only(const nnd_update_block_desc* d, const char* what) {
// ... 125 lines not shown
        const int y = ty0 + (p2 >> 3), xx = tx0 + (p2 & 7);
        tail_bias = bias[f];
        if (y < H && xx < W) {
            const long pix = pix_off(lay, y, xx);
            if (advance == 2) tail_state = flow[(b * FC + f) * HW + pix];
            else if (advance) tail_state = coords[b * HW + pix];
        }
    }
    {
        const int pos = tid & 63, cg = tid >> 6;
        const int gy = ty0 + pos / 10 - 1, gx = tx0 + pos % 10 - 1;
        const bool ok = pos < 60 && gy >= 0 && gy < H && gx >= 0 && gx < W;
        const long off = ok ? pix_off(lay, gy, gx) : 0;
        if (x_c4) {
            for (int q0 = cg; q0 < hid / 4; q0 += 32) {
                float4 v4[4];
#pragma unroll
                for (int j = 0; j < 4; ++j) v4[j] = *reinterpret_cast<const float4*>(src + (long)min(q0 + 8 * j, hid / 4 - 1) * 4 * HW + 4 * off);
#pragma unroll
                for (int j = 0; j < 4; ++j)
                    if (q0 + 8 * j < hid / 4) {
                        float* pp = patch + (q0 + 8 * j) * 4 * 64 + pos;
                        pp[0] = ok ? v4[j].x : 0.f;
                        pp[64] = ok ? v4[j].y : 0.f;
                        pp[128] = ok ? v4[j].z : 0.f;
                        pp[192] = ok ? v4[j].w : 0.f;
                    }
            }
        } else
        for (int c0 = cg; c0 < hid; c0 += 64) {
            float v[8];
#pragma unroll
            for (int j = 0; j < 8; ++j) v[j] = src[(long)min(c0 + 8 * j, hid - 1) * HW + off];
#pragma unroll
            for (int j = 0; j < 8; ++j)
                if (c0 + 8 * j < hid) patch[(c0 + 8 * j) * 64 + pos] = ok ? v[j] : 0.f;
        }
    }
    for (int e = tid; e < FC * hid * 9; e += 512) wl[e] = w[e];
    __syncthreads();
    const int px = tid & 31, slice = tid >> 5;
    const int r = px >> 3, c = px & 7;
    const int cps = hid / 16;
    float acc[FC];
#pragma unroll
    for (int f = 0; f < FC; ++f) acc[f] = 0.f;
    for (int ci = slice * cps; ci < (slice + 1) * cps; ++ci) {
        const float* pp = patch + ci * 64 + r * 10 + c;
#pragma unroll
        for (int t = 0; t < 9; ++t) {
            const float v = pp[(t / 3) * 10 + t % 3];
#pragma unroll
            for (int f = 0; f < FC; ++f) fmac_scalar(acc[f], wl[(f * hid + ci) * 9 + t], v);
        }
    }
#pragma unroll
    for (int f = 0; f < FC; ++f) part[(slice * FC + f) * 32 + px] = acc[f];
    __syncthreads();
    if (tid < 32 * FC) {
        const int f = tid >> 5, p2 = tid & 31;
        float sum = 0.f;
#pragma unroll
        for (int sl = 0; sl < 16; ++sl) sum += part[(sl * FC + f) * 32 + p2];
        sum += tail_bias;
        const int y = ty0 + (p2 >> 3), xx = tx0 + (p2 & 7);
        if (y < H && xx < W) {
            const long pix = pix_off(lay, y, xx);
            delta[(b * FC + f) * HW + pix] = sum;
            if (advance == 2) {
                const float fl = tail_state + sum;
                flow[(b * FC + f) * HW + pix] = fl;
                hx_flow[b * hx_bs + f * (long)hx_cs + pix * hx_pm] = fl;
            } else if (advance) {
                const float cnew = tail_state + sum;
                const float fl = absolute ? cnew : cnew - (float)xx;
                coords[b * HW + pix] = cnew;
                flow[b * HW + pix] = fl;
                hx_flow[b * hx_bs + pix * hx_pm] = fl;
            }
        }
    }
}

static Act act(float* p, int64_t bs, int C) { return Act{p, bs, C}; }

static bool ws_c4() { return !switches().no_c4; }
static int64_t ws_chan(int c, int64_t n) { return ws_c4() ? (int64_t)(c / 4) * 4 * n + c % 4 : (int64_t)c * n; }
static int ws_pm() { return ws_c4() ? 4 : 1; }

static ConvIO conv_io(const Plan& p, const Bufs& w, int id, Act corr, int64_t n , float* mask_dst, float* delta_dst) {
    const int hid = p.d.hidden_dim, ctx = p.d.context_dim, fc = p.d.flow_channels;
    const int hxC = 2 * hid + ctx;
    ConvIO io{};
    switch (id) {
        case C_C1: io.src0 = corr; io.out0 = act(w.c1, 256 * n, 256); break;
        case C_C2: io.src0 = act(w.c1, 256 * n, 256); io.out0 = act(w.cf, 256 * n, 192); break;
        case C_F2: io.src0 = act(w.f1, 128 * n, 128); io.out0 = act(w.cf + 192 * n, 256 * n, 64); break;
        case C_CV: io.src0 = act(w.cf, 256 * n, 256); io.out0 = act(w.hx + (hid + ctx) * n, hxC * n, hid - fc); break;
        case C_ZR1:
        case C_ZR2:
            io.src0 = act(w.hx, hxC * n, hxC);
            io.out0 = act(w.z, hid * n, hid);
            io.out1 = act(w.rh, hid * n, hid);
            io.aux0 = act(w.hx, hxC * n, hid);
            io.hidden = hid;
            break;
        case C_Q1:
        case C_Q2:
            io.src0 = act(w.rh, hid * n, hid);
            io.src1 = act(w.hx + hid * n, hxC * n, ctx + hid);
            io.out0 = act(w.hx, hxC * n, hid);
            io.aux0 = act(w.hx, hxC * n, hid);
            io.aux1 = act(w.z, hid * n, hid);
            break;
        case C_ZR1X:
        case C_ZR2X: {
            io.src0 = act(w.hx, hxC * n, hid);
            io.src1 = act(w.hx + (hid + ctx) * n, hxC * n, hid);
            io.out0 = act(w.z, hid * n, hid);
            io.out1 = act(w.rh, hid * n, hid);
            io.aux0 = act(w.hx, hxC * n, hid);
            io.bmap = act(w.ctxb + (id == C_ZR1X ? 0 : 3 * hid) * n, 6 * hid * n, 2 * hid);
            io.hidden = hid;
            break;
        }
        case C_Q1X:
        case C_Q2X:
            io.src0 = act(w.rh, hid * n, hid);
            io.src1 = act(w.hx + (hid + ctx) * n, hxC * n, hid);
            io.out0 = act(w.hx, hxC * n, hid);
            io.aux0 = act(w.hx, hxC * n, hid);
            io.aux1 = act(w.z, hid * n, hid);
            io.bmap = act(w.ctxb + (id == C_Q1X ? 2 * hid : 5 * hid) * n, 6 * hid * n, hid);
            break;
        case C_ZR1C:
        case C_ZR2C:
            io.src0 = act(w.hx + hid * n, hxC * n, ctx);
            io.out0 = act(w.ctxb + (id == C_ZR1C ? 0 : 3 * hid) * n, 6 * hid * n, 2 * hid);
            break;
        case C_Q1C:
        case C_Q2C:
            io.src0 = act(w.hx + hid * n, hxC * n, ctx);
            io.out0 = act(w.ctxb + (id == C_Q1C ? 2 * hid : 5 * hid) * n, 6 * hid * n, hid);
            break;
        case C_FHM: io.src0 = act(w.hx, hxC * n, hid); io.out0 = act(w.fm, 3 * hid * n, 3 * hid); break;
        case C_M2:
            io.src0 = act(w.fm + hid * n, 3 * hid * n, 2 * hid);
            io.out0 = act(mask_dst, p.d.mask_channels * n, p.d.mask_channels);
            io.scale = 0.25f;
            break;
    }
    io.src_tiled = io.dst_tiled = true;
    if (ws_c4()) {
        switch (id) {
            case C_C1: io.dst_c4 = true; break;
            case C_C2: io.src_c4 = io.dst_c4 = true; break;
            case C_F2: io.dst_c4 = true; break;
            case C_CV: io.src_c4 = io.dst_c4 = true; break;
            case C_FHM: io.src_c4 = io.dst_c4 = true; break;
            case C_M2: io.src_c4 = true; break;
            default: io.src_c4 = io.dst_c4 = true; break;
        }
    }
    return io;
}

static int conv_epi(int id) {
    switch (id) {
        case C_ZR1: case C_ZR2: case C_ZR1X: case C_ZR2X: return EPI_GRU_ZR;
        case C_Q1: case C_Q2: case C_Q1X: case C_Q2X: return EPI_GRU_Q;
        case C_ZR1C: case C_ZR2C: case C_Q1C: case C_Q2C: return EPI_LINEAR;
        case C_M2: return EPI_SCALE;
        default: return EPI_RELU;
    }
}

__global__ void __launch_bounds__(256) lds_poison_kernel(unsigned pattern) {
    extern __shared__ unsigned poison_lds[];
    for (int i = threadIdx.x; i < 160 * 1024 / 4; i += 256) poison_lds[i] = pattern;
    __syncthreads();
    if (poison_lds[(threadIdx.x * 97) % (160 * 1024 / 4)] != pattern) __builtin_trap();
}

static int debug_sync(const char* what, hipStream_t s) {
    if (switches().lds_poison_on) {
        static std::atomic<unsigned> raised{0};
        if (int rc = raise_lds_limit(reinterpret_cast<const void*>(lds_poison_kernel), raised)) return rc;
        hipLaunchKernelGGL(lds_poison_kernel, dim3(2048), dim3(256), 160 * 1024, s, switches().lds_poison);
    }
    if (!switches().debug_sync) return NND_OK;
    fprintf(stderr, "[nnd] %s ...", what);
    fflush(stderr);
    NND_HIP_CHECK(hipStreamSynchronize(s));
    fprintf(stderr, " ok\n");
    fflush(stderr);
    return NND_OK;
}

static int run_conv(const Plan& p, const float* blob, const Bufs& w, int id, Act corr, float* mask_dst, float* delta_dst,
                    int B, int H, int W, hipStream_t s) {
    ConvIO io = conv_io(p, w, id, corr, tiled_plane(H, W), mask_dst, delta_dst);
    int rc = launch_conv(p.L[id], blob, io, conv_epi(id), B, H, W, s);
    if (rc != NND_OK) return rc;
    return debug_sync(kConvNames[id], s);
}

static int run_convf1(const Plan& p, const float* blob, const float* flow, int64_t fbs, float* out, int B, int H, int W,
                      hipStream_t s) {
    const int tiles_x = cdiv(W, 32), tiles_y = cdiv(H, 8);
    dim3 grid(tiles_x * tiles_y, 8, B), block(256);
    const Lay lay = make_lay(H, W, true);
    const int64_t n = lay.plane;
    if (p.d.flow_channels == 1)
        hipLaunchKernelGGL(convf1_kernel<1>, grid, block, 0, s, flow, (long)fbs, blob + p.f1_w, blob + p.f1_b, out, (long)(128 * n), H, W, tiles_x, lay);
    else
        hipLaunchKernelGGL(convf1_kernel<2>, grid, block, 0, s, flow, (long)fbs, blob + p.f1_w, blob + p.f1_b, out, (long)(128 * n), H, W, tiles_x, lay);
    NND_LAUNCH_CHECK();
    return debug_sync("encoder.convf1", s);
}

static int run_fc2(const Plan& p, const float* blob, const Bufs& w, float* delta_dst, int advance, bool absolute, int B, int H,
                   int W, hipStream_t s) {
    const int hid = p.d.hidden_dim, ctx = p.d.context_dim, fc = p.d.flow_channels, hxC = 2 * hid + ctx;
    const Lay lay = make_lay(H, W, true);
    const int64_t n = lay.plane;
    const int tiles_x = cdiv(W, 8);
    dim3 grid(tiles_x * cdiv(H, 4), 1, B), block(512);
    const size_t lds = fc2_lds_bytes(hid, fc);
    NND_REQUIRE(hid % 16 == 0 && lds <= 64 * 1024, "flow_head.conv2: hidden_dim %d not supported", hid);
    NND_REQUIRE(advance != 1 || fc == 1, "flow_head.conv2: the coordinate advance needs flow_channels == 1");
    float* hx_flow = w.hx + ws_chan(hxC - fc, n);
    const int hx_cs = (int)(ws_chan(hxC - fc + 1, n) - ws_chan(hxC - fc, n));
    if (fc == 1)
        hipLaunchKernelGGL(flow_head2_kernel<1>, grid, block, lds, s, w.fm, (long)(3 * hid * n), hid, blob + p.fc2_w, blob + p.fc2_b,
                           delta_dst, w.coords, w.flow, hx_flow, (long)(hxC * n), hx_cs, ws_pm(), ws_c4() ? 1 : 0, H, W, tiles_x, advance, absolute ? 1 : 0, lay);
    else
        hipLaunchKernelGGL(flow_head2_kernel<2>, grid, block, lds, s, w.fm, (long)(3 * hid * n), hid, blob + p.fc2_w, blob + p.fc2_b,
                           delta_dst, w.coords, w.flow, hx_flow, (long)(hxC * n), hx_cs, ws_pm(), ws_c4() ? 1 : 0, H, W, tiles_x, advance == 2 ? 2 : 0, 0, lay);
    NND_LAUNCH_CHECK();
    return debug_sync("flow_head.conv2", s);
}

static int calib_flow_branch(const Plan& p, const float* blob, const Bufs& w, const float* flow, int B, int H, int W, hipStream_t s) {
    if (!calibrating() || !p.L[C_F2].range_scaled()) return NND_OK;
    const int64_t n = tiled_plane(H, W);
    int rc = run_convf1(p, blob, flow, (int64_t)p.d.flow_channels * n, w.f1, B, H, W, s);
    if (rc != NND_OK) return rc;
    return calib_amax_act(Act{w.f1, 128 * n, 128}, make_lay(H, W, true), B, H, W, blob + p.L[C_F2].tail_off(), s);
}

static int run_flow_branch(const Plan& p, const float* blob, const Bufs& w, const float* flow, Act corr, int B, int H, int W,
                           hipStream_t s) {
    const int fc = p.d.flow_channels;
    const int64_t n = tiled_plane(H, W);
    if (flow_branch_supported(p.L[C_F2], fc) && !switches().no_fused_flow_branch) {
        if (int rc0 = calib_flow_branch(p, blob, w, flow, B, H, W, s)) return rc0;
        const ConvIO io = conv_io(p, w, C_F2, corr, n, nullptr, nullptr);
        int rc = launch_flow_branch(p.L[C_F2], blob, blob + p.f1_wt, blob + p.f1_b, flow, (int64_t)fc * n, fc, io, B, H, W, s);
        if (rc != NND_OK) return rc;
        return debug_sync("encoder.convf1+convf2", s);
    }
    int rc = run_convf1(p, blob, flow, (int64_t)fc * n, w.f1, B, H, W, s);
    if (rc != NND_OK) return rc;
    return run_conv(p, blob, w, C_F2, corr, nullptr, nullptr, B, H, W, s);
}

static int run_update(const Plan& p, const float* blob, const Bufs& w, Act corr, const float* flow, float* mask_dst,
                      float* delta_dst, int B, int H, int W, hipStream_t s) {
    int rc;
    NND_TRY(run_conv(p, blob, w, C_C1, corr, nullptr, nullptr, B, H, W, s));
    NND_TRY(run_conv(p, blob, w, C_C2, corr, nullptr, nullptr, B, H, W, s));
    NND_TRY(run_flow_branch(p, blob, w, flow, corr, B, H, W, s));
    NND_TRY(run_conv(p, blob, w, C_CV, corr, nullptr, nullptr, B, H, W, s));
    NND_TRY(run_conv(p, blob, w, C_ZR1, corr, nullptr, nullptr, B, H, W, s));
    NND_TRY(run_conv(p, blob, w, C_Q1, corr, nullptr, nullptr, B, H, W, s));
    if (p.sep) {
        NND_TRY(run_conv(p, blob, w, C_ZR2, corr, nullptr, nullptr, B, H, W, s));
        NND_TRY(run_conv(p, blob, w, C_Q2, corr, nullptr, nullptr, B, H, W, s));
    }
    NND_TRY(run_conv(p, blob, w, C_FHM, corr, nullptr, nullptr, B, H, W, s));
    NND_TRY(run_fc2(p, blob, w, delta_dst, 0, false, B, H, W, s));
    if (mask_dst) NND_TRY(run_conv(p, blob, w, C_M2, corr, mask_dst, nullptr, B, H, W, s));
    return NND_OK;
}

int to_tiled(const float* src, float* dst, int64_t dbs, int B, int C, int H, int W, hipStream_t s, int c0, bool c4) {
    const long total = (long)B * C * H * W;
    hipLaunchKernelGGL(to_tiled_kernel, dim3((unsigned)cdiv64(total, 256)), dim3(256), 0, s, src, dst, (long)dbs, c0, B, C, H, W,
                       make_lay(H, W, true, c4));
    NND_LAUNCH_CHECK();
    return NND_OK;
}
int from_tiled(const float* src, int64_t sbs, float* dst, int B, int C, int H, int W, hipStream_t s, int c0, bool c4) {
    const long total = (long)B * C * H * W;
    hipLaunchKernelGGL(from_tiled_kernel, dim3((unsigned)cdiv64(total, 256)), dim3(256), 0, s, src, (long)sbs, c0, dst, B, C, H, W,
                       make_lay(H, W, true, c4));
    NND_LAUNCH_CHECK();
    return NND_OK;
}


}

using namespace nnd;

extern "C" {

int nnd_update_block_num_tensors(const nnd_update_block_desc* desc) {
    Plan p;
    if (make_plan(desc, &p) != NND_OK) return NND_ERR_INVALID;
    return p.num_tensors;
}

int64_t nnd_update_block_packed_floats(const nnd_update_block_desc* desc) {
    Plan p;
    if (make_plan(desc, &p) != NND_OK) return NND_ERR_INVALID;
    return p.total;
}

int nnd_update_block_pack(const nnd_update_block_desc* desc, const float* const* t, float* out) {
    Plan p;
    int rc = make_plan(desc, &p);
    if (rc != NND_OK) return rc;
    NND_REQUIRE(t && out, "update_block_pack: null pointer");
    for (int i = 0; i < p.num_tensors; ++i) NND_REQUIRE(t[i], "update_block_pack: tensor %d is null", i);
    const int hid = p.d.hidden_dim, fc = p.d.flow_channels;
    memset(out, 0, sizeof(float) * p.total);
    auto one = [&](int id, int ti) {
        const float* w[1] = {t[ti]};
        const float* b[1] = {t[ti + 1]};
        int co[1] = {p.L[id].Cout};
        pack_conv(p.L[id], 1, w, b, co, out);
    };
    auto two = [&](int id, int ta, int tb, int ca, int cb) {
        const float* w[2] = {t[ta], t[tb]};
        const float* b[2] = {t[ta + 1], t[tb + 1]};
        int co[2] = {ca, cb};
        pack_conv(p.L[id], 2, w, b, co, out);
    };
    one(C_C1, 0);
    one(C_C2, 2);
    memcpy(out + p.f1_w, t[4], sizeof(float) * 128 * fc * 49);
    memcpy(out + p.f1_b, t[5], sizeof(float) * 128);
    for (int ch = 0; ch < 128; ++ch)
        for (int k = 0; k < fc * 49; ++k) out[p.f1_wt + (int64_t)k * 128 + ch] = t[4][(int64_t)ch * fc * 49 + k];
    one(C_F2, 6);
    one(C_CV, 8);
    const int ctx = p.d.context_dim, gin = 2 * hid + ctx;
    std::vector<int> map_x(2 * hid), map_c(ctx);
    for (int i = 0; i < hid; ++i) {
        map_x[i] = i;
        map_x[hid + i] = hid + ctx + i;
    }
    for (int i = 0; i < ctx; ++i) map_c[i] = hid + i;
    auto gru = [&](int pass, int tz, int tr, int tq) {
        const int zr = pass == 0 ? C_ZR1 : C_ZR2, q = pass == 0 ? C_Q1 : C_Q2;
        two(zr, tz, tr, hid, hid);
        one(q, tq);
        const float* wzr[2] = {t[tz], t[tr]};
        const float* bzr[2] = {t[tz + 1], t[tr + 1]};
        const float* nob[2] = {nullptr, nullptr};
        int czr[2] = {hid, hid};
        pack_conv(p.L[zr - C_ZR1 + C_ZR1X], 2, wzr, nob, czr, out, map_x.data(), gin);
        pack_conv(p.L[zr - C_ZR1 + C_ZR1C], 2, wzr, bzr, czr, out, map_c.data(), gin);
// ... 132 lines not shown
                          int64_t up_iter_stride, float* low_out, float* net_out, float* workspace, int B, int H, int W,
                          int rate, int iters, void* stream, const float* geo_pyramid = nullptr, int groups = 1,
                          const CreArgs* cre = nullptr, const float* interleaved = nullptr, int flat_groups = 0) {
    Plan p;
    int rc = make_plan(desc, &p);
    if (rc != NND_OK) return rc;
    const bool last_flag = (p.d.flags & NND_FLAG_LAST_UPSAMPLE_ONLY) != 0;
    NND_REQUIRE(!last_flag || up_iter_stride == 0,
                "refine: NND_FLAG_LAST_UPSAMPLE_ONLY writes one upsampled map, so up_iter_stride must be 0 (got %lld)", (long long)up_iter_stride);
    const bool last_only = last_flag && !(p.d.flags & NND_FLAG_CALIBRATE);
    NND_REQUIRE(packed && (pyramid || cre) && net && inp && up_out && workspace, "refine: null pointer");
    const bool igev = geo_pyramid != nullptr;
    const int fc = p.d.flow_channels;
    if (cre) {
        NND_REQUIRE(fc == 2 && p.d.cor_planes == 36, "cre_stereo_refine: needs flow_channels 2 and cor_planes 36");
        NND_REQUIRE(cre->f1 && cre->f2 && (cre->extra || cre->warped), "cre_stereo_refine: null feature map / scratch");
        NND_REQUIRE(cre->extra || cre->warped_floats >= (int64_t)B * cre->C * H * W,
                    "cre_stereo_refine: iter mode needs a scratch of B*C*H*W = %lld floats, got %lld", (long long)B * cre->C * H * W,
                    (long long)cre->warped_floats);
    } else {
        NND_REQUIRE(fc == 1, "raft_stereo_refine: flow_channels must be 1");
        NND_REQUIRE(p.d.cor_planes == num_levels * (2 * radius + 1) * (igev ? 2 * groups : (flat_groups > 0 ? flat_groups : 1)),
                    "refine: cor_planes %d does not match levels*(2r+1)%s", p.d.cor_planes, igev ? "*2*groups" : (flat_groups > 0 ? "*groups" : ""));
        NND_REQUIRE(!(igev && flat_groups > 0), "refine: the IGEV and the group-RAFT lookups exclude each other");
    }

    NND_REQUIRE(p.d.mask_channels == 9 * rate * rate, "raft_stereo_refine: mask_channels %d != 9*rate^2", p.d.mask_channels);
    NND_REQUIRE(B > 0 && H > 0 && W > 0 && iters > 0, "raft_stereo_refine: bad shape");
    CalibScope calib((p.d.flags & NND_FLAG_CALIBRATE) && split_range_scaled(p.d.arithmetic));
    hipStream_t s = (hipStream_t)stream;
    Bufs w;
    carve(p, B, H, W, workspace, &w);
    const int hid = p.d.hidden_dim, ctx = p.d.context_dim, hxC = 2 * hid + ctx;
    const Lay lay = make_lay(H, W, true);
    const int64_t n = lay.plane;
    NND_TRY(to_tiled(net, w.hx, hxC * n, B, hid, H, W, s, 0, ws_c4()));
    NND_TRY(to_tiled(inp, w.hx, hxC * n, B, ctx, H, W, s, hid, ws_c4()));
    float* hx_flow = w.hx + ws_chan(hxC - fc, n);
    const unsigned eg = (unsigned)cdiv64((int64_t)B * H * W, 256);
    if (cre) {
        if (disp_init) {
            NND_TRY(to_tiled(disp_init, w.flow, fc * n, B, fc, H, W, s));
            NND_TRY(to_tiled(disp_init, w.hx, hxC * n, B, fc, H, W, s, hxC - fc, ws_c4()));
        } else {
            NND_HIP_CHECK(hipMemsetAsync(w.flow, 0, sizeof(float) * B * fc * n, s));
            NND_TRY(to_tiled(nullptr, w.hx, hxC * n, B, fc, H, W, s, hxC - fc, ws_c4()));
        }
    } else {
        hipLaunchKernelGGL(init_coords_kernel, dim3(eg), dim3(256), 0, s, w.coords, w.flow, hx_flow, (long)(hxC * n), ws_pm(), disp_init, B, H,
                           W, igev ? 1 : 0, lay);
        NND_LAUNCH_CHECK();
    }
    const bool cre_cl = cre && cre->extra && cre->warped && cre->warped_floats >= 2 * (int64_t)B * cre->C * H * W &&
                        agcl_offset_cl_supported(cre->C) && !switches().agcl_v1;
    if (cre_cl) {
        NND_TRY(nchw_to_nhwc_launch(cre->f1, cre->warped, B, cre->C, H * W, s));
        NND_TRY(nchw_to_nhwc_launch(cre->f2, cre->warped + (int64_t)B * cre->C * H * W, B, cre->C, H * W, s));
    }
    Act c = act(w.corr, p.d.cor_planes * n, p.d.cor_planes);
    auto lookup = [&](hipStream_t st_, int it) -> int {
        if (cre) {
            if (cre->extra && cre_cl)
                return agcl_offset_cl_launch(cre->warped, cre->warped + (int64_t)B * cre->C * H * W, w.flow, cre->extra, w.corr, B, cre->C,
                                             H, W, it & 1, st_, true);
            if (cre->extra) return agcl_offset_launch(cre->f1, cre->f2, w.flow, cre->extra, w.corr, B, cre->C, H, W, it & 1, st_, true);
            return agcl_iter_launch(cre->f1, cre->f2, w.flow, cre->warped, w.corr, B, cre->C, H, W, it & 1, st_, true);
        }
        if (igev) return igev_lookup_launch(pyramid, geo_pyramid, w.coords, w.corr, B, groups, H, W, num_levels, radius, st_, true);
        if (flat_groups > 0) return group_lookup_flat_launch(pyramid, w.coords, w.corr, B, flat_groups, H, W, num_levels, radius, st_, true);
        return corr1d_lookup_launch(pyramid, w.coords, w.corr, B, H, W, num_levels, radius, st_, true);
    };
    for (int id : {(int)C_ZR1C, (int)C_Q1C, (int)C_ZR2C, (int)C_Q2C})
        if (p.sep || id < C_ZR2C) NND_TRY(run_conv(p, packed, w, id, c, nullptr, nullptr, B, H, W, s));
    const bool no_fuse_up = switches().no_fused_upsample;
    const bool no_fuse_lk = switches().no_fused_lookup;
    const bool fused_up = !no_fuse_up && mask_upsample_supported(rate, 2 * hid, fc);
    const bool fold_fh = fused_up && !cre && fc == 1 && mask_upsample_fold_supported(p.L[C_M2], hid) &&
                         (long)B * cdiv(H, 4) * cdiv(W, 8) <= 256 && !switches().no_folded_flow_head;
    float* coords_alt = w.mask;
    float* flow_alt = w.mask + ((int64_t)B * n + 63) / 64 * 64;
    const bool fused_lk = !cre && !no_fuse_lk && flat_groups == 0;
    const bool merged_fbl = fused_lk && !igev && !switches().no_merged_fb_lookup && !switches().no_fused_flow_branch &&
                            flow_branch_supported(p.L[C_F2], fc) && flow_branch_lookup_supported(p.L[C_F2].arith);
    auto loop_conv = [&](int id) -> int {
        probe_mark(id, s);
        const int rc_ = run_conv(p, packed, w, id, c, nullptr, nullptr, B, H, W, s);
        probe_mark(id, s);
        return rc_;
    };
    if (calibrating() && fused_lk && interleaved && p.L[C_C1].range_scaled() && igev_lookup_convc1_il_supported(groups, num_levels, radius))
        NND_TRY(calib_amax_flat(interleaved, nnd_igev_interleaved_floats(B, groups, H, W, num_levels), packed + p.L[C_C1].tail_off(), s));
    for (int it = 0; it < iters; ++it) {
        if (merged_fbl) {
            probe_mark(C_F2, s);
            NND_TRY(calib_flow_branch(p, packed, w, w.flow, B, H, W, s));
            const ConvIO fio = conv_io(p, w, C_F2, c, n, nullptr, nullptr);
            NND_TRY(flow_branch_lookup_launch(p.L[C_F2], packed, packed + p.f1_wt, packed + p.f1_b, w.flow, (int64_t)fc * n, fc, fio, pyramid,
                                              w.coords, p.L[C_C1], w.c1, 256 * n, B, H, W, num_levels, radius, s, ws_c4()));
            NND_TRY(debug_sync("encoder.convf1+convf2 | lookup+convc1", s));
            probe_mark(C_F2, s);
        } else {
        probe_mark(C_F2, s);
        NND_TRY(run_flow_branch(p, packed, w, w.flow, c, B, H, W, s));
        probe_mark(C_F2, s);
        if (fused_lk && interleaved && igev_lookup_convc1_il_supported(groups, num_levels, radius)) {
            NND_TRY(igev_lookup_convc1_il_launch(interleaved, groups, w.coords, p.L[C_C1], packed, w.c1, 256 * n, B, H, W, num_levels,
                                                 radius, s, ws_c4()));
            NND_TRY(debug_sync("lookup+convc1 (interleaved)", s));
        } else if (fused_lk && p.L[C_C1].arith == 0) {
            NND_TRY(lookup_convc1_launch(pyramid, geo_pyramid, groups, w.coords, p.L[C_C1], packed, w.c1, 256 * n, B, H, W,
                                         num_levels, radius, s, ws_c4()));
            NND_TRY(debug_sync("lookup+convc1", s));
        } else {
            NND_TRY(lookup(s, it));
            NND_TRY(debug_sync("lookup", s));
            NND_TRY(run_conv(p, packed, w, C_C1, c, nullptr, nullptr, B, H, W, s));
        }
        }
        NND_TRY(loop_conv(C_C2));
        NND_TRY(loop_conv(C_CV));
        NND_TRY(loop_conv(C_ZR1X));
        NND_TRY(loop_conv(C_Q1X));
        if (p.sep) {
            NND_TRY(loop_conv(C_ZR2X));
            NND_TRY(loop_conv(C_Q2X));
        }
        if (last_only && it + 1 < iters) {
            ConvIO io = conv_io(p, w, C_FHM, c, n, nullptr, nullptr);
            io.cout_need = hid;
            NND_TRY(launch_conv(p.L[C_FHM], packed, io, conv_epi(C_FHM), B, H, W, s));
            NND_TRY(debug_sync("flow_head.conv1", s));
            NND_TRY(run_fc2(p, packed, w, w.delta, cre ? 2 : 1, igev, B, H, W, s));
            continue;
        }
        NND_TRY(loop_conv(C_FHM));
        float* up_it = up_out + (int64_t)it * up_iter_stride;
        if (fold_fh) {
            MaskUpFlowHead fh;
            fh.x = w.fm; fh.xbs = (int64_t)3 * hid * n; fh.hid = hid;
            fh.w = packed + p.fc2_w; fh.bias = packed + p.fc2_b;
            fh.coords_in = w.coords; fh.coords_out = coords_alt; fh.flow_out = flow_alt; fh.delta_out = w.delta;
            fh.hx_flow = hx_flow; fh.hx_bs = (long)(hxC * n); fh.hx_pm = ws_pm(); fh.absolute = igev ? 1 : 0;
            NND_TRY(mask_upsample_launch(p.L[C_M2], packed, w.fm + hid * n, (int64_t)3 * hid * n, w.flow, up_it, B, H, W, rate, s,
                                         true, fc, ws_c4(), &fh));
            NND_TRY(debug_sync("flow_head.conv2 + mask.2 + upsample", s));
            std::swap(w.coords, coords_alt);
            std::swap(w.flow, flow_alt);
            continue;
        }
        NND_TRY(run_fc2(p, packed, w, w.delta, cre ? 2 : 1, igev, B, H, W, s));
        if (fused_up) {
            NND_TRY(mask_upsample_launch(p.L[C_M2], packed, w.fm + hid * n, (int64_t)3 * hid * n, w.flow, up_it, B, H, W, rate, s,
                                         true, fc, ws_c4()));
            NND_TRY(debug_sync("mask.2 + upsample", s));
        } else {
            NND_TRY(run_conv(p, packed, w, C_M2, c, w.mask, nullptr, B, H, W, s));
            NND_TRY(convex_upsample_launch(w.flow, w.mask, up_it, B, fc, H, W, rate, s, true));
            NND_TRY(debug_sync("convex upsample", s));
        }
    }
    if (low_out) NND_TRY(from_tiled(w.flow, fc * n, low_out, B, fc, H, W, s));
    if (net_out) NND_TRY(from_tiled(w.hx, hxC * n, net_out, B, hid, H, W, s, 0, ws_c4()));
    return NND_OK;
}

static int conv2d_layer(int Cout, int Cin, int KH, int KW, int arithmetic, ConvLayer* L, int64_t* total) {
    NND_REQUIRE(Cout > 0 && Cin > 0, "conv2d: bad channel counts");
    NND_REQUIRE(conv_shape_built(KH, KW), "conv2d: kernel %dx%d not built (1x1, 3x3, 1x5, 5x1)", KH, KW);
    NND_REQUIRE(arithmetic == 0 || conv_split_supported(KH, KW, Cin, 1, arithmetic),
                "conv2d: arithmetic %d not built for %dx%d with %d input channels (3 = bf16x3, 2 = fp16x2, 1 = fp16: Cin %% 16 == 0)", arithmetic, KH, KW, Cin);
    int64_t off = 0;
    *L = mk(KH, KW, Cin, Cout, &off, arithmetic);
    if (total) *total = off;
    return NND_OK;
}

int64_t nnd_conv2d_packed_floats_ex(int Cout, int Cin, int KH, int KW, int arithmetic) {
    ConvLayer L;
    int64_t total;
    if (conv2d_layer(Cout, Cin, KH, KW, arithmetic, &L, &total) != NND_OK) return NND_ERR_INVALID;
    return total;
}
int64_t nnd_conv2d_packed_floats(int Cout, int Cin, int KH, int KW) { return nnd_conv2d_packed_floats_ex(Cout, Cin, KH, KW, 0); }

int nnd_conv2d_pack_ex(const float* w_host, const float* b_host, int Cout, int Cin, int KH, int KW, int arithmetic, float* packed_host) {
    ConvLayer L;
    int rc = conv2d_layer(Cout, Cin, KH, KW, arithmetic, &L, nullptr);
    if (rc != NND_OK) return rc;
    NND_REQUIRE(w_host && b_host && packed_host, "conv2d_pack: null pointer");
    const float* w[1] = {w_host};
    const float* b[1] = {b_host};
    int co[1] = {Cout};
    pack_conv(L, 1, w, b, co, packed_host);
    return NND_OK;
}
int nnd_conv2d_pack(const float* w_host, const float* b_host, int Cout, int Cin, int KH, int KW, float* packed_host) {
    return nnd_conv2d_pack_ex(w_host, b_host, Cout, Cin, KH, KW, 0, packed_host);
}

int nnd_conv2d_forward_ex(const float* packed_dev, const float* x, float* y, int B, int Cin, int H, int W, int Cout, int KH,
                          int KW, int relu, int arithmetic, void* stream) {
    ConvLayer L;
    int rc = conv2d_layer(Cout, Cin, KH, KW, arithmetic, &L, nullptr);
    if (rc != NND_OK) return rc;
    NND_REQUIRE(packed_dev && x && y && B > 0 && H > 0 && W > 0, "conv2d_forward: bad argument");
    const int64_t n = (int64_t)H * W;
    ConvIO io{};
    io.src0 = act(const_cast<float*>(x), Cin * n, Cin);
    io.out0 = act(y, Cout * n, Cout);
    return launch_conv(L, packed_dev, io, relu ? EPI_RELU : EPI_LINEAR, B, H, W, (hipStream_t)stream);
}
int nnd_conv2d_calibrate_ex(float* packed_dev, const float* x, int B, int Cin, int H, int W, int Cout, int KH, int KW, int arithmetic,
                            int32_t* status_dev, void* stream) {
    ConvLayer L;
    int rc = conv2d_layer(Cout, Cin, KH, KW, arithmetic, &L, nullptr);
    if (rc != NND_OK) return rc;
    NND_REQUIRE(packed_dev && x && B > 0 && H > 0 && W > 0, "conv2d_calibrate: bad argument");
    if (!L.range_scaled()) return NND_OK;
    const int64_t n = (int64_t)H * W;
    rc = calib_amax_act(act(const_cast<float*>(x), Cin * n, Cin), make_lay(H, W, false), B, H, W, packed_dev + L.tail_off(), (hipStream_t)stream);
    if (rc != NND_OK) return rc;
    const int64_t off = L.tail_off();
    return calib_finish(packed_dev, &off, 1, status_dev, (hipStream_t)stream);
}

int nnd_conv2d_scale_slots_ex(int Cout, int Cin, int KH, int KW, int arithmetic, int64_t* offsets, int n) {
    ConvLayer L;
    int rc = conv2d_layer(Cout, Cin, KH, KW, arithmetic, &L, nullptr);
    if (rc != NND_OK) return rc;
    if (!offsets) return 1;
    NND_REQUIRE(n >= 1, "conv2d_scale_slots: room for %d offsets, a layer has 1 slot", n);
    offsets[0] = L.range_scaled() ? L.tail_off() : -1;
    return 1;
// ... 280 lines not shown
```

Before: 138.0 pairs/s.

## Fuse flow-head conv2 tap projection into conv1 epilogue via per-tap partial sums

Inside the split-arithmetic conv kernel for flow_head.conv1, the ReLU output of the first hid channels is projected onto the 3x3 conv2 weights per tap. The per-tap partial sums are reduced through LDS and written as a small map (hid/32 * 9 * fc planes) instead of the full hidden activation. flow_head.conv2 then becomes a cheap per-pixel gather that sums the 9 shifted taps and adds the bias, removing the second large 3x3 conv over hid channels. In exchange the conv kernel uses more LDS and does extra epilogue FMAs and a barrier. A new NG=4 finish path is also added.

```diff
diff --git a/nndepth_amd/csrc/common.h b/nndepth_amd/csrc/common.h
--- a/nndepth_amd/csrc/common.h
+++ b/nndepth_amd/csrc/common.h
@@ -56,6 +56,7 @@
     int split_ny, split_ks, split_p;
     bool split_no_fast;
     bool no_merged_fb_lookup;
+    bool no_fh_tapsum;
     int conv_p, conv_ks, conv_wco;
     int agcl_pb;
     bool lds_poison_on;
@@ -158,7 +159,12 @@
     bool dst_c4 = false;
     int cout_need = 0;
     int force_ks = 0;
-};
+    const float* tap_w = nullptr;
+    Act tap_s{};
+    int tap_hid = 0, tap_fc = 0;
+};
+
+static inline int64_t tap_map_channels(int hid, int fc) { return (int64_t)(hid / 32) * 9 * fc; }
 
 static inline bool conv_shape_built(int KH, int KW) { return (KH == 1 && (KW == 1 || KW == 5)) || (KW == 1 && KH == 5) || (KH == 3 && KW == 3); }
 
@@ -228,6 +234,9 @@
     long hx_bs;
     int hx_pm;
     int absolute;
+    const float* s;
+    long s_bs;
+    int planes;
 };
 
 bool mask_upsample_supported(int rate, int cin, int flow_channels);
diff --git a/nndepth_amd/csrc/conv_epilogue.h b/nndepth_amd/csrc/conv_epilogue.h
--- a/nndepth_amd/csrc/conv_epilogue.h
+++ b/nndepth_amd/csrc/conv_epilogue.h
@@ -29,6 +29,11 @@
     const float* cscale;
     float scale;
     int dbg_stamp;
+    const float* tap_w;
+    float* tap_s;
+    long tap_bs;
+    int tap_hid, tap_fc;
+    int tap_lds;
 };
 
 __device__ __forceinline__ float exp_acc(float x) {
@@ -306,7 +311,7 @@
 
 template <int P, int NG>
 __device__ __forceinline__ void epi_c4_store(const ConvArgs& a, const float4 (&cacc)[P][NG], const int cb, const int b, const int h2,
-                                             const int q0, const EpiOpsC4<P, NG>& e) {
+                                             const int q0, const EpiOpsC4<P, NG>& e, const int skip_below = 0) {
     const long DP = a.ld.plane;
     const int epi = a.epi;
     auto get = [](const float4& v, int i) { return i == 0 ? v.x : (i == 1 ? v.y : (i == 2 ? v.z : v.w)); };
@@ -317,7 +322,7 @@
 #pragma unroll
         for (int j = 0; j < NG; ++j) {
             const int co0 = cb * 32 + 8 * (q0 + j) + 4 * h2;
-            if (co0 >= a.Cout) continue;
+            if (co0 >= a.Cout || co0 < skip_below) continue;
             const bool full = co0 + 3 < a.Cout;
             float r0[4], r1[4];
 #pragma unroll
@@ -367,6 +372,76 @@
     }
 }
 
+template <int P, int NG>
+__device__ __forceinline__ void epi_planar_relu_store(const ConvArgs& a, const float4 (&cacc)[P][NG], const int cb, const int b, const int h2,
+                                                      const int q0, const EpiOpsC4<P, NG>& e) {
+    auto get = [](const float4& v, int i) { return i == 0 ? v.x : (i == 1 ? v.y : (i == 2 ? v.z : v.w)); };
+#pragma unroll
+    for (int pp = 0; pp < P; ++pp) {
+        if (!e.pix_ok[pp]) continue;
+#pragma unroll
+        for (int j = 0; j < NG; ++j)
+#pragma unroll
+            for (int i = 0; i < 4; ++i) {
+                const int co = cb * 32 + 8 * (q0 + j) + 4 * h2 + i;
+                if (co < a.Cout) a.out0[b * a.obs0 + co * a.ld.plane + e.pix[pp]] = relu_nan(get(cacc[pp][j], i) + get(e.bm[pp][j], i));
+            }
+    }
+}
+template <int P, int NG, int FC>
+__device__ __forceinline__ void tap_partial(const float4 (&cacc)[P][NG], const EpiOpsC4<P, NG>& e, const float* wl_cb, const int wfs, const int h2,
+                                            const int q0, float* tp_wave, const int pxl) {
+    auto get = [](const float4& v, int i) { return i == 0 ? v.x : (i == 1 ? v.y : (i == 2 ? v.z : v.w)); };
+#pragma unroll
+    for (int pp = 0; pp < P; ++pp)
+#pragma unroll
+        for (int f = 0; f < FC; ++f) {
+            float part[9];
+#pragma unroll
+            for (int t = 0; t < 9; ++t) part[t] = 0.f;
+#pragma unroll
+            for (int j = 0; j < NG; ++j) {
+                const float4* wp = reinterpret_cast<const float4*>(wl_cb + f * wfs + (8 * (q0 + j) + 4 * h2) * 9);
+                float4 w[9];
+#pragma unroll
+                for (int k = 0; k < 9; ++k) w[k] = wp[k];
+#pragma unroll
+                for (int i = 0; i < 4; ++i) {
+                    const float v = relu_nan(get(cacc[pp][j], i) + get(e.bm[pp][j], i));
+#pragma unroll
+                    for (int t = 0; t < 9; ++t) fmac_scalar(part[t], get(w[(i * 9 + t) >> 2], (i * 9 + t) & 3), v);
+                }
+                __builtin_amdgcn_sched_barrier(0);
+            }
+#pragma unroll
+            for (int t = 0; t < 9; ++t) {
+                const float s = part[t] + __shfl_xor(part[t], 32, 64);
+                if (h2 == 0) tp_wave[(pp * 9 * FC + f * 9 + t) * 32 + pxl] = s;
+            }
+            __builtin_amdgcn_sched_barrier(0);
+        }
+}
+template <int P, int FC>
+__device__ __forceinline__ void tap_store(const ConvArgs& a, const float* tp, const int cb0, const int ncbh, const int ks, const int b,
+                                          const int tile0, const int tid, const int nthreads) {
+    constexpr int NTF = 9 * FC;
+    const int total = ncbh * P * NTF * 32;
+    for (int e = tid; e < total; e += nthreads) {
+        const int px = e & 31;
+        int rest = e >> 5;
+        const int tf = rest % NTF;
+        rest /= NTF;
+        const int pp = rest % P, cbi = rest / P;
+        const float* src = tp + ((size_t)(cbi * ks * P + pp) * NTF + tf) * 32 + px;
+        float sum = src[0];
+        for (int k = 1; k < ks; ++k) sum += src[(size_t)k * P * NTF * 32];
+        const int t = tile0 + pp;
+        if (t >= a.npos) continue;
+        const int y = (t / a.tiles_x) * 4 + (px >> 3), x = (t % a.tiles_x) * 8 + (px & 7);
+        if (y < a.H && x < a.W) a.tap_s[b * a.tap_bs + ((long)(cb0 + cbi) * NTF + tf) * a.ld.plane + (long)t * 32 + px] = sum;
+    }
+}
+
 template <int P>
 __device__ __forceinline__ void conv_epilogue(const ConvArgs& a, const f32x16 (&acc)[P], const int cb, const int b, const int h2,
                                               const int reg0, const int nreg, const int (&ys)[P], const int (&xs)[P]) {
diff --git a/nndepth_amd/csrc/conv_launch.h b/nndepth_amd/csrc/conv_launch.h
--- a/nndepth_amd/csrc/conv_launch.h
+++ b/nndepth_amd/csrc/conv_launch.h
@@ -3,6 +3,7 @@
 #include "conv_epilogue.h"
 #include "layout.h"
 
+#include <cstdint>
 #include <cstring>
 
 namespace nnd {
@@ -17,6 +18,10 @@
     NND_REQUIRE(!io.dst_c4 || (io.dst_tiled && (L.Cout % 4 == 0 || (!io.bmap.ptr && !io.aux0.ptr && !io.aux1.ptr && !io.out1.ptr))),
                 "%s: c4 destination with per-pixel operands needs Cout %% 4 == 0", who);
     NND_REQUIRE(epi != EPI_AFFINE || L.s_off >= 0, "%s: EPI_AFFINE needs a packed scale vector", who);
+    NND_REQUIRE(!io.tap_w || (io.tap_s.ptr && epi == EPI_RELU && io.dst_tiled && !io.bmap.ptr && L.KH == 3 && L.KW == 3 && L.stride == 1 &&
+                              (io.tap_fc == 1 || io.tap_fc == 2) && io.tap_hid > 0 && io.tap_hid % 32 == 0 && io.tap_hid <= L.Cout &&
+                              reinterpret_cast<uintptr_t>(io.tap_w) % 16 == 0),
+                "%s: the tap projection needs a 3x3 stride-1 ReLU conv with a tile-major destination, 1 or 2 flow channels, hid %% 32 == 0 and 16-B aligned weights", who);
     return NND_OK;
 }
 
@@ -35,6 +40,7 @@
     a.ld = make_lay(H, W, io.dst_tiled, io.dst_c4);
     a.H = H; a.W = W; a.Hin = Hin; a.Win = Win; a.Cout = L.Cout; a.nchunks = L.nchunks; a.epi = epi; a.hidden = io.hidden; a.flags = io.flags;
     a.cscale = L.s_off >= 0 ? blob + L.s_off : nullptr; a.scale = io.scale;
+    a.tap_w = io.tap_w; a.tap_s = io.tap_s.ptr; a.tap_bs = io.tap_s.bstride; a.tap_hid = io.tap_hid; a.tap_fc = io.tap_fc;
 }
 
 template <class CanStage>
diff --git a/nndepth_amd/csrc/conv_mfma.hip b/nndepth_amd/csrc/conv_mfma.hip
--- a/nndepth_amd/csrc/conv_mfma.hip
+++ b/nndepth_amd/csrc/conv_mfma.hip
@@ -517,6 +517,7 @@
     }
     int rc, Hin, Win;
     NND_TRY(conv_check_io("conv", L, io, epi, H, W, &Hin, &Win));
+    NND_REQUIRE(!io.tap_w, "conv: the tap projection is built on the split arithmetics only");
     NND_REQUIRE(io.src1.C == 0 || io.src0.C % L.CI_T == 0, "conv: first source (%d ch) must be a multiple of %d", io.src0.C, L.CI_T);
     NND_REQUIRE(!io.src_c4 || L.stride == 1, "conv: c4 sources need stride 1");
     NND_REQUIRE((long)(L.Cin + 2 * L.CI_T) * tiled_plane(Hin, Win) < (1L << 31), "conv: plane offsets exceed 32 bits");
diff --git a/nndepth_amd/csrc/conv_split.hip b/nndepth_amd/csrc/conv_split.hip
--- a/nndepth_amd/csrc/conv_split.hip
+++ b/nndepth_amd/csrc/conv_split.hip
@@ -2,6 +2,7 @@
 #include "conv_split_kernel.h"
 #include "flow_branch.h"
 
+#include <algorithm>
 #include <atomic>
 #include <cmath>
 #include <cstdlib>
@@ -159,6 +160,11 @@
     ConvArgs a;
     conv_fill_args(L, blob, io, epi, H, W, Hin, Win, &a);
     a.tiles_x = cfg.tiles_x; a.wco = cfg.wco; a.ks = cfg.ks; a.npos = cfg.ntiles;
+    if (io.tap_w) {
+        a.tap_lds = (int)cfg.lds;
+        cfg.lds += (size_t)std::min(cfg.wco, io.tap_hid / 32) * (cfg.ks * cfg.P * 9 * io.tap_fc * 32 + io.tap_fc * 288) * sizeof(float);
+        NND_REQUIRE(cfg.lds <= 160 * 1024, "conv_split: the tap projection needs %zu bytes of LDS (at most 163840)", cfg.lds);
+    }
 #ifdef NND_DBG_STAMPS
     {
         static std::atomic<int> launches{0};
diff --git a/nndepth_amd/csrc/conv_split_kernel.h b/nndepth_amd/csrc/conv_split_kernel.h
--- a/nndepth_amd/csrc/conv_split_kernel.h
+++ b/nndepth_amd/csrc/conv_split_kernel.h
@@ -98,8 +98,9 @@
     static constexpr bool ON = NT >= 5 && P == 2;
 };
 
-template <int KH, int KW, int NS, int P, int NU, bool FAST, bool SRC4, int AD_, int MAXT, int STR = 1>
+template <int KH, int KW, int NS, int P, int NU, bool FAST, bool SRC4, int AD_, int MAXT, int STR = 1, int TAPFC = 0>
 __global__ void __launch_bounds__(MAXT) conv_split_kernel(ConvArgs a) {
+    static_assert(TAPFC == 0 || (KH * KW == 9 && STR == 1), "tap projection: the stride-1 3x3 kernels");
     static_assert(STR == 1 || (FAST && (KH * KW == 9 || KH * KW == 1)), "stride 2: 3x3 / 1x1, FAST regime");
     using Geo = SplitGeom<KH, KW, NS, STR>;
     constexpr int NT = KH * KW, PH = KH / 2, PW = KW / 2;
@@ -179,6 +180,18 @@
         if constexpr (PIPE) goff[i] = cho[i] * (int)SP + (int)pix_off(a.ls, min(max(gy, 0), Hin - 1), min(max(gx, 0), Win - 1));
     }
 
+    constexpr int TAPWN = TAPFC == 0 ? 1 : (TAPFC * 72 + 63) / 64;
+    const int tap_cb0 = blockIdx.y * wco, tap_ncbh = min(wco, max(0, a.tap_hid / 32 - tap_cb0));
+    float4 tapw_r[TAPWN];
+    if constexpr (TAPFC > 0) {
+        const int per_f = tap_ncbh * 72;
+#pragma unroll
+        for (int i = 0; i < TAPWN; ++i) {
+            const int e = min(tid + i * nthreads, TAPFC * per_f - 1), f = per_f > 0 ? e / per_f : 0;
+            tapw_r[i] = per_f > 0 ? reinterpret_cast<const float4*>(a.tap_w + ((long)f * a.tap_hid + tap_cb0 * 32) * 9)[e - f * per_f]
+                                  : make_float4(0.f, 0.f, 0.f, 0.f);
+        }
+    }
     NND_PSTAMP(5);
     f32x16 acc[P];
 #pragma unroll
@@ -280,6 +293,12 @@
     load_x(0);
     NND_PSTAMP(6);
     store_x(0);
+    if constexpr (TAPFC > 0) {
+        float4* wl4 = reinterpret_cast<float4*>(lds_raw + a.tap_lds) + (size_t)tap_ncbh * ks * (P * 9 * TAPFC * 8);
+#pragma unroll
+        for (int i = 0; i < TAPWN; ++i)
+            if (tid + i * nthreads < TAPFC * tap_ncbh * 72) wl4[tid + i * nthreads] = tapw_r[i];
+    }
     NND_PSTAMP(7);
     __syncthreads();
     NND_SSTAMP(1);
@@ -484,7 +503,7 @@
     }
     float* red_all = reinterpret_cast<float*>(lds_raw);
     constexpr int TS = P * 1024;
-    auto exchange = [&]() {
+    auto exchange_write = [&]() {
         if (active) {
             float* red = red_all + (size_t)(cbi * ks + kj) * TS + lane;
 #pragma unroll
@@ -492,42 +511,71 @@
 #pragma unroll
                 for (int reg = 0; reg < 16; ++reg) red[pp * 1024 + reg * 64] = acc[pp][reg];
         }
+    };
+    auto exchange = [&]() {
+        exchange_write();
         __syncthreads();
     };
-    auto finish_c4 = [&](auto ng_c) {
+    constexpr bool tap = TAPFC > 0;
+    auto tap_finish = [&](auto ng_c, auto fc_c, const auto& cacc, const auto& eo) {
+        constexpr int NG = decltype(ng_c)::value, FC = decltype(fc_c)::value;
+        float* tp = reinterpret_cast<float*>(lds_raw + a.tap_lds);
+        const float* wl = tp + (size_t)tap_ncbh * ks * (P * 9 * FC * 32);
+        if (active && cb * 32 < a.tap_hid)
+            tap_partial<P, NG, FC>(cacc, eo, wl + cbi * 288, tap_ncbh * 288, h2, kj * NG, tp + (size_t)(cbi * ks + kj) * (P * 9 * FC * 32), pxl);
+        __syncthreads();
+        tap_store<P, FC>(a, tp, tap_cb0, tap_ncbh, ks, b, blockIdx.x * P, tid, nthreads);
+    };
+    auto finish_c4 = [&](auto ng_c, auto fc_c) {
         constexpr int NG = decltype(ng_c)::value;
+        constexpr int FC = decltype(fc_c)::value;
         const int q0 = kj * NG;
         EpiOpsC4<P, NG> eo;
 #ifndef NND_SPLIT_NO_EPI
         if (active) epi_c4_load<P, NG>(a, cb, b, h2, q0, ys, xs, eo);
 #endif
-        exchange();
-        if (!active) return;
+        if (NG < 4) exchange();
         float4 cacc[P][NG];
-#pragma unroll
-        for (int pp = 0; pp < P; ++pp)
-#pragma unroll
-            for (int j = 0; j < NG; ++j) {
-                float v[4];
-#pragma unroll
-                for (int i = 0; i < 4; ++i) {
-                    const float* red = red_all + (size_t)(cbi * ks) * TS + pp * 1024 + (4 * (q0 + j) + i) * 64 + lane;
-                    float sum = red[0];
-#pragma unroll
-                    for (int sl = 1; sl < 4 / NG; ++sl) sum += red[(size_t)sl * TS];
-                    v[i] = sum;
+        if (active) {
+#pragma unroll
+            for (int pp = 0; pp < P; ++pp)
+#pragma unroll
+                for (int j = 0; j < NG; ++j) {
+                    float v[4];
+#pragma unroll
+                    for (int i = 0; i < 4; ++i) {
+                        if constexpr (NG == 4) {
+                            v[i] = acc[pp][4 * j + i];
+                        } else {
+                            const float* red = red_all + (size_t)(cbi * ks) * TS + pp * 1024 + (4 * (q0 + j) + i) * 64 + lane;
+                            float sum = red[0];
+#pragma unroll
+                            for (int sl = 1; sl < 4 / NG; ++sl) sum += red[(size_t)sl * TS];
+                            v[i] = sum;
+                        }
+                    }
+                    cacc[pp][j] = make_float4(v[0], v[1], v[2], v[3]);
                 }
-                cacc[pp][j] = make_float4(v[0], v[1], v[2], v[3]);
-            }
-        NND_SSTAMP(3);
+            NND_SSTAMP(3);
 #ifdef NND_SPLIT_NO_EPI
-        if (cacc[0][0].x != 123.456f) return;
-#endif
-        epi_c4_store<P, NG>(a, cacc, cb, b, h2, q0, eo);
-    };
-    if (a.ld.ci == 4) {
-        if (ks == 4) finish_c4(std::integral_constant<int, 1>{});
-        else if (ks == 2) finish_c4(std::integral_constant<int, 2>{});
+            if (cacc[0][0].x != 123.456f) return;
+#endif
+            if (FC > 0 && a.ld.ci != 4) {
+                if (cb * 32 >= a.tap_hid) epi_planar_relu_store<P, NG>(a, cacc, cb, b, h2, q0, eo);
+            } else {
+                epi_c4_store<P, NG>(a, cacc, cb, b, h2, q0, eo, FC > 0 ? a.tap_hid : 0);
+            }
+        }
+        if constexpr (FC > 0) tap_finish(ng_c, fc_c, cacc, eo);
+    };
+    auto finish_c4_tap = [&](auto ng_c) {
+        if constexpr (tap) finish_c4(ng_c, std::integral_constant<int, TAPFC>{});
+        else if constexpr (decltype(ng_c)::value < 4) finish_c4(ng_c, std::integral_constant<int, 0>{});
+    };
+    if (a.ld.ci == 4 || tap) {
+        if (ks == 4) finish_c4_tap(std::integral_constant<int, 1>{});
+        else if (ks == 2) finish_c4_tap(std::integral_constant<int, 2>{});
+        else if (tap) finish_c4_tap(std::integral_constant<int, 4>{});
         else {
             if (!active) return;
             NND_SSTAMP(3);
@@ -577,9 +625,9 @@
 
 inline int split_tiles(int H, int W, int* tiles_x) { return (*tiles_x = cdiv(W, 8)) * cdiv(H, 4); }
 
-template <int KH, int KW, int NS, int P, int NU, bool FAST, bool SRC4, int AD, int MAXT, int STR = 1>
+template <int KH, int KW, int NS, int P, int NU, bool FAST, bool SRC4, int AD, int MAXT, int STR = 1, int TAPFC = 0>
 int launch_split_kernel(const ConvArgs& a, dim3 grid, dim3 block, size_t lds, hipStream_t stream) {
-    auto kern = conv_split_kernel<KH, KW, NS, P, NU, FAST, SRC4, AD, MAXT, STR>;
+    auto kern = conv_split_kernel<KH, KW, NS, P, NU, FAST, SRC4, AD, MAXT, STR, TAPFC>;
     if ((int)block.x > MAXT) {
         set_error("conv_split: %u threads exceed the %d-thread bound of this instantiation", block.x, MAXT);
         return NND_ERR_INVALID;
@@ -602,15 +650,27 @@
 #endif
 }
 
-template <int KH, int KW, int NS, bool FAST, bool SRC4, int STR>
+template <int KH, int KW, int NS, bool FAST, bool SRC4, int STR, int TAPFC = 0>
 int launch_split_nu(const ConvArgs& a, const SplitCfg& cfg, hipStream_t stream) {
     constexpr int AD = FAST ? split_fast_ad<KH, KW, NS>() : 1;
-    if (split_nu_variant(cfg.nu) == 2) return launch_split_kernel<KH, KW, NS, 2, 2, FAST, SRC4, AD, 768, STR>(a, cfg.grid, cfg.block, cfg.lds, stream);
-    return launch_split_kernel<KH, KW, NS, 2, 4, FAST, SRC4, AD, 768, STR>(a, cfg.grid, cfg.block, cfg.lds, stream);
+    if (split_nu_variant(cfg.nu) == 2) return launch_split_kernel<KH, KW, NS, 2, 2, FAST, SRC4, AD, 768, STR, TAPFC>(a, cfg.grid, cfg.block, cfg.lds, stream);
+    return launch_split_kernel<KH, KW, NS, 2, 4, FAST, SRC4, AD, 768, STR, TAPFC>(a, cfg.grid, cfg.block, cfg.lds, stream);
+}
+template <int KH, int KW, int NS, int TAPFC>
+int launch_split_tap(const ConvArgs& a, const SplitCfg& cfg, hipStream_t stream) {
+    if constexpr (KH * KW == 9) {
+        if (cfg.stride != 1) return NND_ERR_UNSUPPORTED;
+        if (!cfg.fast) return launch_split_nu<KH, KW, NS, false, false, 1, TAPFC>(a, cfg, stream);
+        return a.ls.ci == 4 ? launch_split_nu<KH, KW, NS, true, true, 1, TAPFC>(a, cfg, stream)
+                            : launch_split_nu<KH, KW, NS, true, false, 1, TAPFC>(a, cfg, stream);
+    } else {
+        return NND_ERR_UNSUPPORTED;
+    }
 }
 template <int KH, int KW, int NS>
 int launch_split_shape(const ConvArgs& a, const SplitCfg& cfg, hipStream_t stream) {
     if (cfg.P != 2) return NND_ERR_UNSUPPORTED;
+    if (a.tap_w) return a.tap_fc == 1 ? launch_split_tap<KH, KW, NS, 1>(a, cfg, stream) : launch_split_tap<KH, KW, NS, 2>(a, cfg, stream);
     const bool src4 = a.ls.ci == 4;
     if (cfg.stride == 2) {
         if constexpr (KH * KW == 9 || KH * KW == 1) {
diff --git a/nndepth_amd/csrc/error.cpp b/nndepth_amd/csrc/error.cpp
--- a/nndepth_amd/csrc/error.cpp
+++ b/nndepth_amd/csrc/error.cpp
@@ -33,6 +33,7 @@
     if (const char* e = getenv("NND_SPLIT_CFG")) sscanf(e, "%d,%d,%d", &s.split_ny, &s.split_ks, &s.split_p);
     s.split_no_fast = on("NND_SPLIT_NO_FAST");
     s.no_merged_fb_lookup = on("NND_NO_MERGED_FB_LOOKUP");
+    s.no_fh_tapsum = on("NND_NO_FH_TAPSUM");
     s.conv_p = s.conv_ks = s.conv_wco = -1;
     if (const char* e = getenv("NND_CONV_CFG")) sscanf(e, "%d,%d,%d", &s.conv_p, &s.conv_ks, &s.conv_wco);
     if (const char* e = getenv("NND_CONV_P")) s.conv_p = atoi(e);
diff --git a/nndepth_amd/csrc/fh_tap.h b/nndepth_amd/csrc/fh_tap.h
--- /dev/null
+++ b/nndepth_amd/csrc/fh_tap.h
@@ -0,0 +1,30 @@
+#pragma once
+#include "layout.h"
+
+namespace nnd {
+
+__device__ __forceinline__ float fh_tap_delta(const float* __restrict__ s, const int planes, const int fc, const int f, const float bias,
+                                              const int y, const int x, const int H, const int W, const Lay& lay) {
+    const long n = lay.plane, ps = 9L * fc * n;
+    long off[9];
+    bool in[9];
+#pragma unroll
+    for (int t = 0; t < 9; ++t) {
+        const int yy = y + t / 3 - 1, xx = x + t % 3 - 1;
+        in[t] = yy >= 0 && yy < H && xx >= 0 && xx < W;
+        off[t] = (f * 9 + t) * n + pix_off(lay, min(max(yy, 0), H - 1), min(max(xx, 0), W - 1));
+    }
+    double v[9];
+#pragma unroll
+    for (int t = 0; t < 9; ++t) v[t] = (double)s[off[t]];
+    for (int pl = 1; pl < planes; ++pl) {
+#pragma unroll
+        for (int t = 0; t < 9; ++t) v[t] += (double)s[pl * ps + off[t]];
+    }
+    double acc = in[0] ? v[0] : 0.0;
+#pragma unroll
+    for (int t = 1; t < 9; ++t) acc += in[t] ? v[t] : 0.0;
+    return (float)(acc + (double)bias);
+}
+
+}
diff --git a/nndepth_amd/csrc/mask_upsample.hip b/nndepth_amd/csrc/mask_upsample.hip
--- a/nndepth_amd/csrc/mask_upsample.hip
+++ b/nndepth_amd/csrc/mask_upsample.hip
@@ -1,6 +1,7 @@
 #include "common.h"
 
 #include <type_traits>
+#include "fh_tap.h"
 #include "layout.h"
 #include "split_arith.h"
 
@@ -77,15 +78,9 @@
     }
 
     float fh_state = 0.f, fh_bias = 0.f;
-    auto fh_finish = [&](float* fbase, int t0) {
-        if (t0 >= 60) return;
-        const float* part = fbase + a.fh.hid * 105;
+    auto fh_write = [&](int t0, float sum) {
         const int pr = t0 / 10, pc = t0 % 10;
         const int y = ty0 + pr - 1, x = tx0 + pc - 1;
-        float sum = 0.f;
-#pragma unroll
-        for (int sl = 0; sl < 16; ++sl) sum += part[sl * 64 + t0];
-        sum += fh_bias;
         const bool in = y >= 0 && y < H && x >= 0 && x < W;
         const float cnew = fh_state + sum;
         const float fl = a.fh.absolute ? cnew : cnew - (float)x;
@@ -98,6 +93,15 @@
             a.fh.hx_flow[b * a.fh.hx_bs + pix * a.fh.hx_pm] = fl;
         }
     };
+    auto fh_finish = [&](float* fbase, int t0) {
+        if (t0 >= 60) return;
+        const float* part = fbase + a.fh.hid * 105;
+        float sum = 0.f;
+#pragma unroll
+        for (int sl = 0; sl < 16; ++sl) sum += part[sl * 64 + t0];
+        sum += fh_bias;
+        fh_write(t0, sum);
+    };
     constexpr int NQ4 = (CIN / 4 * 32 + NT - 1) / NT;
     float4 v4[SPLIT ? NQ4 : 1];
     if constexpr (SPLIT) {
@@ -116,7 +120,25 @@
             }
         }
     }
-    if constexpr (FHW > 0) {
+    if constexpr (FHW == 1) {
+        if (tid >= NT) {
+            const int t0 = tid - NT;
+            float sum = 0.f;
+            if (t0 < 60) {
+                const int y = ty0 + t0 / 10 - 1, x = tx0 + t0 % 10 - 1;
+                if (y >= 0 && y < H && x >= 0 && x < W) {
+                    fh_state = a.fh.coords_in[b * XP + pix_off(a.lay, y, x)];
+                    sum = fh_tap_delta(a.fh.s + b * a.fh.s_bs, a.fh.planes, 1, 0, a.fh.bias[0], y, x, H, W, a.lay);
+                }
+            }
+            __builtin_amdgcn_s_barrier();
+            if (t0 < 60) fh_write(t0, sum);
+            __syncthreads();
+            __syncthreads();
+            __syncthreads();
+            return;
+        }
+    } else if constexpr (FHW > 0) {
         if (tid >= NT) {
             float* fbase = lds + Cfg::LDS_FLOATS;
             const int hid = a.fh.hid, fw_ = __builtin_amdgcn_readfirstlane((tid - NT) >> 6), cn = hid / FHW, c0 = fw_ * cn;
@@ -419,13 +441,14 @@
 }
 
 constexpr int MU_FHW = 4;
+constexpr int MU_FHW_TAP = 1;
 template <int RATE, int CIN, int NS, int FHW>
 static int launch_mu_fhw(MaskUpArgs a, int B, hipStream_t stream) {
     using Cfg = MaskUpCfg<RATE, CIN>;
     auto kern = mask_upsample_kernel<RATE, CIN, NS, FHW>;
     a.lds_floats = Cfg::LDS_FLOATS;
     const int fh_floats = a.fh.x ? a.fh.hid * (96 + 9) + 16 * 64 : 0;
-    if (FHW > 0) a.lds_floats = Cfg::LDS_FLOATS + fh_floats + 128;
+    if (FHW > 1) a.lds_floats = Cfg::LDS_FLOATS + fh_floats + 128;
     const size_t lds = a.lds_floats * sizeof(float);
     if (lds > 64 * 1024) {
         static std::atomic<unsigned> raised{0};
@@ -439,7 +462,7 @@
 template <int RATE, int CIN, int NS = 0>
 static int launch_mu(const MaskUpArgs& a, int B, hipStream_t stream) {
     if (a.fh.x) {
-        if constexpr (split_range_scaled(NS)) return launch_mu_fhw<RATE, CIN, NS, MU_FHW>(a, B, stream);
+        if constexpr (split_range_scaled(NS)) return a.fh.s ? launch_mu_fhw<RATE, CIN, NS, MU_FHW_TAP>(a, B, stream) : launch_mu_fhw<RATE, CIN, NS, MU_FHW>(a, B, stream);
         else NND_REQUIRE(false, "mask_upsample: the folded flow head is built for the fp16x2 and fp16 arithmetics");
     }
     return launch_mu_fhw<RATE, CIN, NS, 0>(a, B, stream);
@@ -469,6 +492,7 @@
         NND_REQUIRE(flow_channels == 1 && mask_upsample_fold_supported(L, fh->hid) && fh->w && fh->bias && fh->coords_in && fh->coords_out && fh->flow_out &&
                         fh->delta_out && fh->hx_flow && fh->coords_in != fh->coords_out,
                     "mask_upsample: folded flow head needs one flow channel, hid %% 16 == 0 and distinct old / new state buffers");
+        NND_REQUIRE(!fh->s || (fh->planes > 0 && fh->planes * 32 == fh->hid), "mask_upsample: the tap projection holds hid / 32 plane sets");
         a.fh = *fh;
     }
     if (L.arith == 3) {
diff --git a/nndepth_amd/csrc/update_block.hip b/nndepth_amd/csrc/update_block.hip
--- a/nndepth_amd/csrc/update_block.hip
+++ b/nndepth_amd/csrc/update_block.hip
@@ -1,5 +1,6 @@
 #include "common.h"
 #include "conv_layer.h"
+#include "fh_tap.h"
 #include "layout.h"
 
 #include <cstdlib>
@@ -291,13 +292,47 @@
     }
 }
 
+__global__ void __launch_bounds__(64) flow_head2_tap_kernel(const float* __restrict__ S, long sbs, int planes, int fc, const float* __restrict__ bias,
+                                                            float* __restrict__ delta, float* __restrict__ coords, float* __restrict__ flow,
+                                                            float* __restrict__ hx_flow, long hx_bs, int hx_cs, int hx_pm, int H, int W,
+                                                            int advance, int absolute, Lay lay) {
+    const long HW = lay.plane;
+    const long idx = (long)blockIdx.x * 64 + threadIdx.x;
+    if (idx >= fc * HW) return;
+    const int f = (int)(idx / HW), b = blockIdx.z;
+    const long pix = idx % HW;
+    const int tile = (int)(pix >> 5), y = (tile / lay.TX) * 4 + (int)((pix >> 3) & 3), xx = (tile % lay.TX) * 8 + (int)(pix & 7);
+    if (y >= H || xx >= W) return;
+    float state = 0.f;
+    if (advance == 2) state = flow[(b * fc + f) * HW + pix];
+    else if (advance) state = coords[b * HW + pix];
+    const float sum = fh_tap_delta(S + b * sbs, planes, fc, f, bias[f], y, xx, H, W, lay);
+    delta[(b * fc + f) * HW + pix] = sum;
+    if (advance == 2) {
+        const float fl = state + sum;
+        flow[(b * fc + f) * HW + pix] = fl;
+        hx_flow[b * hx_bs + f * (long)hx_cs + pix * hx_pm] = fl;
+    } else if (advance) {
+        const float cnew = state + sum;
+        const float fl = absolute ? cnew : cnew - (float)xx;
+        coords[b * HW + pix] = cnew;
+        flow[b * HW + pix] = fl;
+        hx_flow[b * hx_bs + pix * hx_pm] = fl;
+    }
+}
+
 static Act act(float* p, int64_t bs, int C) { return Act{p, bs, C}; }
 
 static bool ws_c4() { return !switches().no_c4; }
 static int64_t ws_chan(int c, int64_t n) { return ws_c4() ? (int64_t)(c / 4) * 4 * n + c % 4 : (int64_t)c * n; }
 static int ws_pm() { return ws_c4() ? 4 : 1; }
 
-static ConvIO conv_io(const Plan& p, const Bufs& w, int id, Act corr, int64_t n , float* mask_dst, float* delta_dst) {
+static bool fh_tap_on(const Plan& p) { return p.L[C_FHM].arith != 0 && !switches().no_fh_tapsum; }
+static Act fh_tap_map(const Plan& p, const Bufs& w, int64_t n) {
+    return Act{w.fm, 3 * p.d.hidden_dim * n, (int)tap_map_channels(p.d.hidden_dim, p.d.flow_channels)};
+}
+
+static ConvIO conv_io(const Plan& p, const Bufs& w, int id, Act corr, int64_t n , float* mask_dst, float* delta_dst, const float* tap_w = nullptr) {
     const int hid = p.d.hidden_dim, ctx = p.d.context_dim, fc = p.d.flow_channels;
     const int hxC = 2 * hid + ctx;
     ConvIO io{};
@@ -352,7 +387,16 @@
             io.src0 = act(w.hx + hid * n, hxC * n, ctx);
             io.out0 = act(w.ctxb + (id == C_Q1C ? 2 * hid : 5 * hid) * n, 6 * hid * n, hid);
             break;
-        case C_FHM: io.src0 = act(w.hx, hxC * n, hid); io.out0 = act(w.fm, 3 * hid * n, 3 * hid); break;
+        case C_FHM:
+            io.src0 = act(w.hx, hxC * n, hid);
+            io.out0 = act(w.fm, 3 * hid * n, 3 * hid);
+            if (tap_w) {
+                io.tap_w = tap_w;
+                io.tap_s = fh_tap_map(p, w, n);
+                io.tap_hid = hid;
+                io.tap_fc = fc;
+            }
+            break;
         case C_M2:
             io.src0 = act(w.fm + hid * n, 3 * hid * n, 2 * hid);
             io.out0 = act(mask_dst, p.d.mask_channels * n, p.d.mask_channels);
@@ -407,8 +451,8 @@
 }
 
 static int run_conv(const Plan& p, const float* blob, const Bufs& w, int id, Act corr, float* mask_dst, float* delta_dst,
-                    int B, int H, int W, hipStream_t s) {
-    ConvIO io = conv_io(p, w, id, corr, tiled_plane(H, W), mask_dst, delta_dst);
+                    int B, int H, int W, hipStream_t s, bool fh_tap = false) {
+    ConvIO io = conv_io(p, w, id, corr, tiled_plane(H, W), mask_dst, delta_dst, (fh_tap && id == C_FHM) ? blob + p.fc2_w : nullptr);
     int rc = launch_conv(p.L[id], blob, io, conv_epi(id), B, H, W, s);
     if (rc != NND_OK) return rc;
     return debug_sync(kConvNames[id], s);
@@ -429,11 +473,22 @@
 }
 
 static int run_fc2(const Plan& p, const float* blob, const Bufs& w, float* delta_dst, int advance, bool absolute, int B, int H,
-                   int W, hipStream_t s) {
+                   int W, hipStream_t s, bool fh_tap = false) {
     const int hid = p.d.hidden_dim, ctx = p.d.context_dim, fc = p.d.flow_channels, hxC = 2 * hid + ctx;
     const Lay lay = make_lay(H, W, true);
     const int64_t n = lay.plane;
     const int tiles_x = cdiv(W, 8);
+    if (fh_tap) {
+        NND_REQUIRE(advance != 1 || fc == 1, "flow_head.conv2: the coordinate advance needs flow_channels == 1");
+        float* hxf = w.hx + ws_chan(hxC - fc, n);
+        const int hcs = (int)(ws_chan(hxC - fc + 1, n) - ws_chan(hxC - fc, n));
+        const long items = (long)fc * n;
+        hipLaunchKernelGGL(flow_head2_tap_kernel, dim3((unsigned)cdiv64(items, 64), 1, B), dim3(64), 0, s, (const float*)fh_tap_map(p, w, n).ptr,
+                           (long)fh_tap_map(p, w, n).bstride, hid / 32, fc, blob + p.fc2_b, delta_dst, w.coords, w.flow, hxf, (long)(hxC * n), hcs,
+                           ws_pm(), H, W, fc == 1 ? advance : (advance == 2 ? 2 : 0), (fc == 1 && absolute) ? 1 : 0, lay);
+        NND_LAUNCH_CHECK();
+        return debug_sync("flow_head.conv2", s);
+    }
     dim3 grid(tiles_x * cdiv(H, 4), 1, B), block(512);
     const size_t lds = fc2_lds_bytes(hid, fc);
     NND_REQUIRE(hid % 16 == 0 && lds <= 64 * 1024, "flow_head.conv2: hidden_dim %d not supported", hid);
@@ -487,8 +542,8 @@
         NND_TRY(run_conv(p, blob, w, C_ZR2, corr, nullptr, nullptr, B, H, W, s));
         NND_TRY(run_conv(p, blob, w, C_Q2, corr, nullptr, nullptr, B, H, W, s));
     }
-    NND_TRY(run_conv(p, blob, w, C_FHM, corr, nullptr, nullptr, B, H, W, s));
-    NND_TRY(run_fc2(p, blob, w, delta_dst, 0, false, B, H, W, s));
+    NND_TRY(run_conv(p, blob, w, C_FHM, corr, nullptr, nullptr, B, H, W, s, fh_tap_on(p)));
+    NND_TRY(run_fc2(p, blob, w, delta_dst, 0, false, B, H, W, s, fh_tap_on(p)));
     if (mask_dst) NND_TRY(run_conv(p, blob, w, C_M2, corr, mask_dst, nullptr, B, H, W, s));
     return NND_OK;
 }
@@ -787,9 +842,10 @@
     const bool fused_lk = !cre && !no_fuse_lk && flat_groups == 0;
     const bool merged_fbl = fused_lk && !igev && !switches().no_merged_fb_lookup && !switches().no_fused_flow_branch &&
                             flow_branch_supported(p.L[C_F2], fc) && flow_branch_lookup_supported(p.L[C_F2].arith);
+    const bool fh_tap = fh_tap_on(p);
     auto loop_conv = [&](int id) -> int {
         probe_mark(id, s);
-        const int rc_ = run_conv(p, packed, w, id, c, nullptr, nullptr, B, H, W, s);
+        const int rc_ = run_conv(p, packed, w, id, c, nullptr, nullptr, B, H, W, s, fh_tap);
         probe_mark(id, s);
         return rc_;
     };
@@ -831,19 +887,22 @@
             NND_TRY(loop_conv(C_Q2X));
         }
         if (last_only && it + 1 < iters) {
-            ConvIO io = conv_io(p, w, C_FHM, c, n, nullptr, nullptr);
+            ConvIO io = conv_io(p, w, C_FHM, c, n, nullptr, nullptr, fh_tap ? packed + p.fc2_w : nullptr);
             io.cout_need = hid;
             NND_TRY(launch_conv(p.L[C_FHM], packed, io, conv_epi(C_FHM), B, H, W, s));
             NND_TRY(debug_sync("flow_head.conv1", s));
-            NND_TRY(run_fc2(p, packed, w, w.delta, cre ? 2 : 1, igev, B, H, W, s));
+            NND_TRY(run_fc2(p, packed, w, w.delta, cre ? 2 : 1, igev, B, H, W, s, fh_tap));
             continue;
         }
         NND_TRY(loop_conv(C_FHM));
         float* up_it = up_out + (int64_t)it * up_iter_stride;
         if (fold_fh) {
-            MaskUpFlowHead fh;
+            MaskUpFlowHead fh{};
             fh.x = w.fm; fh.xbs = (int64_t)3 * hid * n; fh.hid = hid;
             fh.w = packed + p.fc2_w; fh.bias = packed + p.fc2_b;
+            if (fh_tap) {
+                fh.s = fh_tap_map(p, w, n).ptr; fh.s_bs = (long)fh_tap_map(p, w, n).bstride; fh.planes = hid / 32;
+            }
             fh.coords_in = w.coords; fh.coords_out = coords_alt; fh.flow_out = flow_alt; fh.delta_out = w.delta;
             fh.hx_flow = hx_flow; fh.hx_bs = (long)(hxC * n); fh.hx_pm = ws_pm(); fh.absolute = igev ? 1 : 0;
             NND_TRY(mask_upsample_launch(p.L[C_M2], packed, w.fm + hid * n, (int64_t)3 * hid * n, w.flow, up_it, B, H, W, rate, s,
@@ -853,7 +912,7 @@
             std::swap(w.flow, flow_alt);
             continue;
         }
-        NND_TRY(run_fc2(p, packed, w, w.delta, cre ? 2 : 1, igev, B, H, W, s));
+        NND_TRY(run_fc2(p, packed, w, w.delta, cre ? 2 : 1, igev, B, H, W, s, fh_tap));
         if (fused_up) {
             NND_TRY(mask_upsample_launch(p.L[C_M2], packed, w.fm + hid * n, (int64_t)3 * hid * n, w.flow, up_it, B, H, W, rate, s,
                                          true, fc, ws_c4()));
```

Result: no change. 138.4 pairs/s (median of 3 runs) (+0.3%).
